# toverainc/willow-inference-server

Hardware: AMD Instinct MI355X
Metric: realtime_multiple (audio_ms / infer_ms), Whisper large-v2 beam=5, 3.84 s clip (higher is better)
Workload: dtype f16; 1 GPU; whisper-large beam=5 clip=3sec (3840 ms) batch=1/GPU, PCM resident in HBM -> ids on host; parallelism=1 independent replicas (utterance sharding, no data-path collective)

## Files before the change

### include/wis_hip.h

```cpp
#ifndef WIS_HIP_H
#define WIS_HIP_H

#include <stddef.h>
#include <stdint.h>

#ifdef __cplusplus
extern "C" {
#endif

#define WIS_ABI_VERSION 1

#define WIS_OK             0
#define WIS_E_ARG         -1
#define WIS_E_FORMAT      -2
#define WIS_E_NOMEM       -3
#define WIS_E_CHECKSUM    -4
#define WIS_E_HIP         -5
#define WIS_E_STATE       -6
#define WIS_E_UNSUPPORTED -7

#define WIS_SAMPLE_RATE 16000
#define WIS_N_FFT       400
#define WIS_HOP         160
#define WIS_N_MELS      80
// ... 38 lines not shown
  const int32_t* suppress_ids;       int32_t n_suppress;
  const int32_t* suppress_ids_begin; int32_t n_suppress_begin;
  const int32_t* lang_ids;           int32_t n_lang;
  int32_t decoder_weight_bits;
} wis_config_t;

#define WIS_DT_F32 0
#define WIS_DT_F16 1
typedef struct {
  const char* name;
  int32_t     dtype;
  int32_t     rank;
  int64_t     shape[4];
  uint64_t    offset;
} wis_tensor_t;

int  wis_model_create(const wis_config_t* cfg, const void* arena, size_t arena_bytes,
                      int arena_on_device, const wis_tensor_t* tensors, int n_tensors,
                      int device, wis_model_t** out);
void wis_model_destroy(wis_model_t* m);
size_t wis_model_device_bytes(const wis_model_t* m);
int  wis_model_clone(wis_model_t* parent, wis_model_t** out);

#define WIS_IN_MEL_HOST 0
#define WIS_IN_MEL_DEV  1
#define WIS_IN_PCM_HOST 2
#define WIS_IN_PCM_DEV  3

typedef struct {
  int32_t input_kind;
  int32_t beam_size;
  int32_t max_new_tokens;
  float   length_penalty;
  float   patience;
  int32_t suppress_blank;
  int32_t suppress_default;
  int32_t fixed_new_tokens;
  int32_t queue_depth;
  int32_t timestamps;
  int32_t max_initial_timestamp_index;
  int32_t no_speech_prob;
  float   repetition_penalty;
  int32_t no_repeat_ngram_size;
} wis_gen_opts_t;

int wis_generate(wis_model_t* m, const float* input, int B, const int32_t* prompt, int P,
                 const wis_gen_opts_t* opts, int32_t* out_ids, int32_t* out_len, float* out_score);

int wis_generate_draft(wis_model_t* m, const float* input, const int32_t* prompt, int P, const wis_gen_opts_t* opts,
                       const int32_t* draft, int n_draft, int32_t* out_ids, int32_t* out_len, float* out_score, int32_t* accepted);

int wis_generate_draft_beam(wis_model_t* m, const float* input, const int32_t* prompt, int P, const wis_gen_opts_t* opts,
                            const int32_t* draft_tok, const int32_t* draft_org, int n_steps,
                            int32_t* out_ids, int32_t* out_len, float* out_score, int32_t* accepted_steps);
int wis_last_trajectory(wis_model_t* m, int b, int32_t* tok, int32_t* org, int cap_steps, int32_t* n_steps);

int wis_last_no_speech_prob(wis_model_t* m, int B, float* out);

int wis_detect_language(wis_model_t* m, const float* input, int input_kind, int B, float* lang_probs);

int wis_debug_encode(wis_model_t* m, const float* input, int input_kind, int B, float* enc_out);
int wis_debug_logits(wis_model_t* m, const float* input, int input_kind, int B,
                     const int32_t* dec_in, int T, float* logits);
int wis_debug_logits_rows(wis_model_t* m, const float* input, int input_kind, int B,
                          const int32_t* dec_in, int T, int R, float* logits);
int wis_model_set_alignment_heads(wis_model_t* m, const int32_t* layer_head_pairs, int n);
int wis_align(wis_model_t* m, const float* input, int input_kind, int B, const int32_t* start_seq, int P,
              const int32_t* text, const int32_t* text_len, const int32_t* num_frames, int median_filter_width,
              int32_t* path_text, int32_t* path_time, int32_t* path_len, float* token_probs);
int wis_debug_align_matrix(wis_model_t* m, const float* input, int input_kind, int B, const int32_t* start_seq, int P,
                           const int32_t* text, const int32_t* text_len, const int32_t* num_frames, int median_filter_width, float* out);
int wis_align_last_timing(wis_model_t* m, float* ms);
int wis_op_dtw(int device, const float* x, int N, int M, int32_t* text_idx, int32_t* time_idx, int32_t* len);
int wis_op_align_matrix(int device, const float* q, const void* kx_f16, int T_tokens, int n_heads_sel, int T, int frames, int width, float* out);
int wis_debug_tree_logits(wis_model_t* m, const float* input, int input_kind, const int32_t* prompt, int P, int beam,
                          const int32_t* tok, const int32_t* org, int n_steps, float* logits);

int wis_debug_search(wis_model_t* m, const float* logits, int n_steps, int B, const wis_gen_opts_t* opts,
                     int32_t* out_ids, int32_t* out_len, float* out_score, int32_t* out_finish_step, int32_t* out_parent);

int wis_debug_handoff(wis_model_t* m, int raise_flag, int* retries, int* spin_disabled);

typedef struct {
  float logmel_ms, encoder_ms, crosskv_ms, prefill_ms, decode_ms, total_ms;
  int32_t decode_steps;
  int32_t decode_steps_needed;
} wis_timing_t;
int wis_last_timing(const wis_model_t* m, wis_timing_t* t);

int wis_debug_phase_cycles(wis_model_t* m, int B, int beam, int pos, uint64_t* out);

int wis_debug_timeline(wis_model_t* m, int B, int beam, int pos, int use_graph, uint64_t* out, int n_out);
int wis_debug_sampling_cycles(wis_model_t* m, uint64_t* out);

int wis_bench_weight_stream(wis_model_t* m, int M, int passes, float* total_ms, int* launches_per_pass,
                            double* bytes_per_pass);

int wis_dev_alloc(int device, size_t bytes, void** out);
int wis_dev_free(int device, void* p);
int wis_dev_h2d(int device, void* dst, const void* src, size_t bytes);
int wis_dev_d2h(int device, void* dst, const void* src, size_t bytes);
int wis_dev_sync(int device);
int wis_dev_copy_peer(int dst_device, void* dst, int src_device, const void* src, size_t bytes);

int wis_op_gemm(int device, const void* A_f16, int lda, const void* W_f16, const float* bias,
                const float* residual, void* C, int M, int N, int K, int flags);
int wis_op_layernorm(int device, const float* x, const float* gamma, const float* beta,
                     void* y_f16, int M, int d);
int wis_op_enc_attention(int device, const void* qk_f16, const void* vt_f16, void* out_f16,
                         int B, int T, int Tpad, int H);
int wis_op_enc_attention_ex(int device, const void* qk_f16, const void* vt_f16, void* out_f16,
                            int B, int T, int Tpad, int H, int form);
int wis_op_gemv(int device, const void* x, const float* gamma, const float* beta,
                const void* W_f16, const float* bias, void* y, int M, int N, int K, int flags);
int wis_op_gemv_cols(int device, const void* x_f16, const void* W_f16, const float* bias, void* y, void* y16,
                     int M, int N, int K, int flags, int cols);

int wis_op_dec_self_attn(int device, const float* q, const void* kc_f16, const void* vc_f16, const int32_t* pos, void* out_f16,
                         int M, int H, int ctx, int rpu, int sstride, int rmul);
int wis_op_dec_cross_attn(int device, const float* q, const void* kx_f16, const void* vt_f16, void* out_f16,
                          int B, int R, int H, int T, int chunks);
int wis_op_dec_cross_attn_folded(int device, const float* q_raw, const float* xres, const float* qcs, const float* qb,
                                 const void* kx_f16, const void* vt_f16, void* out_f16, int B, int R, int H, int T, int chunks);

int wis_op_dec_cross_attn_stat(int device, const float* q, const float* q2, const float* stat, const float* qcs, const float* qb,
                               const void* kx_f16, const void* vt_f16, void* out_f16, int B, int R, int H, int T, int chunks,
                               int out_mb, int kv_shared, int no_spin);
int wis_op_dec_self_attn_ex(int device, const float* q, const void* kc_f16, const void* vc_f16, const int32_t* pos, void* out_f16,
                            int M, int H, int ctx, int rpu, int sstride, int rmul, int nb, int out_mb,
                            const int32_t* anc, int w0, int aw, const int32_t* base);
int wis_op_gemv_qkv(int device, const float* x, const float* gamma, const float* beta, const void* W_f16, const float* bias,
                    const int32_t* slot, const int32_t* pos, float* q, void* kc_f16, void* vc_f16, int M, int d, int ctx);
int wis_op_gemv_out_cq(int device, const void* a_f16, const float* x0, const void* Wo_f16, const float* bo, const void* Wq_f16, const float* bq,
                       const float* gamma, const float* beta, float* x1, float* stat, float* q, float* q2, float* qcs, float* qb,
                       int M, int d, int force_frag);

int wis_op_mel_to_image(int device, const float* mel, void* img_f16, int B, int n_mels);
int wis_op_enc_conv(int device, int which, const void* img_f16, const void* W, int w_is_f16, const float* bias, const float* pos, void* out,
                    int B, int T, int Cin, int N);
int wis_op_enc_qkv(int device, const void* xn_f16, const void* W_f16, const float* bias, void* qk_f16, void* vt_f16, int B, int T, int H);
int wis_op_enc_crosskv(int device, const void* mem_f16, const void* W_f16, const float* bias, void* kx_f16, void* vt_f16, int B, int T, int H, int L,
                       int64_t kx_lstride, int64_t vt_lstride);
int wis_op_gemm_splitk_ln(int device, const void* A_f16, const void* W_f16, const float* bias, float* X, const float* gamma, const float* beta,
                          void* Y_f16, int M, int N, int K, int splits);

int wis_op_kv_reorder(int device, void* kc_f16, void* vc_f16, int64_t layer_stride_elems, int L, const int32_t* parent, const int32_t* step_u,
                      const int32_t* done, int B, int beam, int P, int ctx, int d);
int wis_op_kv_gather(int device, void* kc_f16, void* vc_f16, int64_t layer_stride_elems, int L, const int32_t* vstate, const int32_t* done,
                     int beam, int w0, int ctx, int d);
int wis_op_no_speech(int device, const float* logits, int ld, int B, int rs, int r0, int V, int ns, float* out);
int wis_op_lang_probs(int device, const float* logits, int ld, const int32_t* lang_ids, int n_lang, float* probs, int B);
int wis_op_greedy_rows(int device, const float* logits, int n_vocab, int n_vocab_pad, int eot, const float* bias_all, const float* bias_begin,
                       const int32_t* step_u, int B, int beam, int lr_b, int lr_j, int lr_off, const int32_t* rowmap, int32_t* tok_out, float* lp_out);

typedef struct wis_sv wis_sv_t;
typedef struct {
  int32_t conv_dim;
  int32_t n_conv_layers;
  int32_t conv_kernel[8], conv_stride[8];
  int32_t hidden_size, n_heads, n_layers, intermediate_size;
  int32_t num_conv_pos_embeddings, num_conv_pos_embedding_groups;
  int32_t num_buckets, max_bucket_distance;
  int32_t n_tdnn;
  int32_t tdnn_dim[8], tdnn_kernel[8], tdnn_dilation[8];
  int32_t xvector_output_dim;
  int64_t max_samples;
} wis_sv_config_t;
int    wis_sv_create(const wis_sv_config_t* cfg, const void* arena, size_t arena_bytes, int arena_on_device,
                     const wis_tensor_t* tensors, int n_tensors, int device, wis_sv_t** out);
void   wis_sv_destroy(wis_sv_t* sv);
size_t wis_sv_device_bytes(const wis_sv_t* sv);
int    wis_sv_embed(wis_sv_t* sv, const float* pcm, int64_t n, float* emb);
int    wis_sv_rel_buckets(int num_buckets, int max_distance, int first, int n, int32_t* out);
int    wis_debug_sv_taps(wis_sv_t* sv, const float* pcm, int64_t n, int tap, int layer, float* out, int64_t cap_floats,
                         int32_t* rows, int32_t* cols);
int    wis_op_sv_conv0(int device, const float* pcm, int64_t n, const float* w0, const float* gamma, const float* beta, void* y_f16);
int    wis_op_sv_posconv(int device, const float* x, const void* W_f16, const float* bias, float* out, int T);
int    wis_op_sv_attention(int device, const void* qkv_f16, const float* xin, const float* gw, const float* gb, const float* gconst,
                           const float* tab, int L, void* out_f16, int T);
int    wis_op_sv_layernorm(int device, const void* x, int in_f16, const float* gamma, const float* beta, void* y16, float* y32,
                           float* ws, void* ws16, float wl, int wmode, int M, int d);
int    wis_op_sv_xvector_tail(int device, const float* z, int ldz, int T, int n, const float* W_fe, const float* b_fe,
                              float* stats, float* emb);

#ifdef __cplusplus
}
#endif
#endif
```

### willow-inference-server_amd/csrc/dec_kernels.hip

```cpp
#include <string.h>
#include "common.hpp"
#include "kernels.hpp"

namespace wis {

__global__ void pack_gemv_kernel(const f16* __restrict__ W, f16* __restrict__ Wp, int N, int Npad, int K, int n_scale, float scale, int rows) {
  const int ksteps = K / 32;
  const size_t total = (size_t)Npad * ksteps * 4;
  for (size_t idx = (size_t)blockIdx.x * blockDim.x + threadIdx.x; idx < total; idx += (size_t)gridDim.x * blockDim.x) {
    const int row = (int)(idx % rows);
    size_t t = idx / rows;
    const int kq = (int)(t & 3); t >>= 2;
    const int ks = (int)(t % ksteps), nt = (int)(t / ksteps);
    const int n = rows * nt + row, k = 32 * ks + 8 * kq;
    f16x8 v;
    if (n < N) {
      v = *reinterpret_cast<const f16x8*>(W + (size_t)n * K + k);
      if (n < n_scale) {
#pragma unroll
        for (int j = 0; j < 8; ++j) v[j] = (f16)((float)v[j] * scale);
      }
    } else {
#pragma unroll
      for (int j = 0; j < 8; ++j) v[j] = (f16)0.f;
// ... 1744 lines not shown
      if (tid == 0) tl_end(prof);
      return;
    }
    if (pub) {
#pragma unroll
      for (int blk = 0; blk < NB; ++blk)
#pragma unroll
        for (int r4 = 0; r4 < 4; ++r4) own[l15][dhb + 16 * blk + r4] = o_[blk][r4];
      if (wave == NKW && kq == 0) { own[l15][64] = Mc; own[l15][65] = Lc; }
    }
    __syncthreads();
    stamp(pf, 5);
    for (int item = tid; item < R * 32; item += NTHR) {
      const int r = item >> 5, dp = item & 31;
      float2 ml[CM], ov[CM];
      unsigned spins = 0;
      for (;;) {
        bool ok = true;
#pragma unroll
        for (int cc = 0; cc < CM - 1; ++cc) {
          if (cc < C - 1) {
            const gran_t* gp = gbase + ((size_t)cc * 8 + r) * 66;
            const gran_t g0 = ld_gran(gp + 64), g1 = ld_gran(gp + 65), g2 = ld_gran(gp + 2 * dp), g3 = ld_gran(gp + 2 * dp + 1);
            ok = ok & ((unsigned)(g0 >> 32) == tag) & ((unsigned)(g1 >> 32) == tag) & ((unsigned)(g2 >> 32) == tag) & ((unsigned)(g3 >> 32) == tag);
            ml[cc] = make_float2(__uint_as_float((unsigned)g0), __uint_as_float((unsigned)g1));
            ov[cc] = make_float2(__uint_as_float((unsigned)g2), __uint_as_float((unsigned)g3));
          }
        }
        if (ok) break;
        if (++spins > CA_SPIN_LIMIT) { atomicOr(epoch, 1u); break; }
        __builtin_amdgcn_s_sleep(1);
      }
      float M_ = own[r][64];
#pragma unroll
      for (int cc = 0; cc < CM - 1; ++cc) if (cc < C - 1) M_ = fmaxf(M_, ml[cc].x);
      float L = 0.f, O0 = 0.f, O1 = 0.f;
#pragma unroll
      for (int cc = 0; cc < CM - 1; ++cc) {
        if (cc < C - 1) {
          const float w = __expf(ml[cc].x - M_);
          L = fmaf(ml[cc].y, w, L); O0 = fmaf(ov[cc].x, w, O0); O1 = fmaf(ov[cc].y, w, O1);
        }
      }
      {
        const float w = __expf(own[r][64] - M_);
        L = fmaf(own[r][65], w, L); O0 = fmaf(own[r][2 * dp], w, O0); O1 = fmaf(own[r][2 * dp + 1], w, O1);
      }
      const float inv = 1.0f / L;
      typedef _Float16 f16x2 __attribute__((ext_vector_type(2)));
      const f16x2 o2 = {(f16)(O0 * inv), (f16)(O1 * inv)};
      *reinterpret_cast<f16x2*>(out + (out_mb ? xf_index(b * R + r, h * 64 + 2 * dp, out_mb) : (size_t)(b * R + r) * d + h * 64 + 2 * dp)) = o2;
    }
    if (tid == 0) __hip_atomic_store(epoch + 1 + b * H + h, tag, __ATOMIC_RELAXED, __HIP_MEMORY_SCOPE_AGENT);
    stamp(pf, 6);
    if (tid == 0) tl_end(prof);
    return;
  }
  float* pbase = part + ((size_t)(b * H + h) * C) * R * 66;
  if (pub) {
    float* pp = pbase + ((size_t)c * R + l15) * 66;
#pragma unroll
    for (int blk = 0; blk < NB; ++blk)
#pragma unroll
      for (int r4 = 0; r4 < 4; ++r4) st_sc1(pp + dhb + 16 * blk + r4, o_[blk][r4]);
    if (wave == NKW && kq == 0) { st_sc1(pp + 64, Mc); st_sc1(pp + 65, Lc); }
  }
  asm volatile("s_waitcnt vmcnt(0)" ::: "memory");
  __syncthreads();
  stamp(pf, 5);
  if (tid == 0) {
    const unsigned prev = __hip_atomic_fetch_add(counters + b * H + h, 1u, __ATOMIC_RELAXED, __HIP_MEMORY_SCOPE_AGENT);
    const int last = (prev == (unsigned)(C - 1));
    if (last) {
      __hip_atomic_store(counters + b * H + h, 0u, __ATOMIC_RELAXED, __HIP_MEMORY_SCOPE_AGENT);
      __builtin_amdgcn_fence(__ATOMIC_ACQUIRE, "agent");
    }
    s_last = last;
  }
  __syncthreads();
  if (tid == 0) tl_end(prof);
  if (!s_last) return;
  for (int item = tid; item < R * 32; item += NTHR) {
    const int r = item >> 5, dp = item & 31;
    float2 ml[CM], ov[CM];
#pragma unroll
    for (int cc = 0; cc < CM; ++cc) {
      if (cc < C) {
        const float* pp = pbase + ((size_t)cc * R + r) * 66;
        ml[cc] = *reinterpret_cast<const float2*>(pp + 64);
        ov[cc] = *reinterpret_cast<const float2*>(pp + 2 * dp);
      }
    }
    float M_ = -INFINITY;
#pragma unroll
    for (int cc = 0; cc < CM; ++cc) if (cc < C) M_ = fmaxf(M_, ml[cc].x);
    float L = 0.f, O0 = 0.f, O1 = 0.f;
#pragma unroll
    for (int cc = 0; cc < CM; ++cc) {
      if (cc < C) {
        const float w = __expf(ml[cc].x - M_);
        L = fmaf(ml[cc].y, w, L); O0 = fmaf(ov[cc].x, w, O0); O1 = fmaf(ov[cc].y, w, O1);
      }
    }
    const float inv = 1.0f / L;
    typedef _Float16 f16x2 __attribute__((ext_vector_type(2)));
    const f16x2 o2 = {(f16)(O0 * inv), (f16)(O1 * inv)};
    *reinterpret_cast<f16x2*>(out + (out_mb ? xf_index(b * R + r, h * 64 + 2 * dp, out_mb) : (size_t)(b * R + r) * d + h * 64 + 2 * dp)) = o2;
  }
  stamp(pf, 6);
}

int launch_dec_cross_attn(hipStream_t st, const CrossAttnP& p) {
  const int B = p.B, R = p.R, H = p.H, d = p.d, T = p.T, Tpad = p.Tpad, chunks = p.chunks, xres_is_stat = p.xres_is_stat;
  const float* const xres = p.xres;
  if (xres && (!p.qcs || !p.qb || R > 8 || d > (xres_is_stat ? 2048 : 1280))) { set_error("dec_cross_attn: folded query needs column sums, bias, R <= 8 and d <= 1280 (2048 from partials)"); return WIS_E_ARG; }
  if (xres_is_stat && !xres) { set_error("dec_cross_attn: the fold from partials needs the row partials"); return WIS_E_ARG; }
  if (R < 1 || R > 16 || chunks < 1 || chunks > 16) { set_error("dec_cross_attn: R=%d chunks=%d unsupported", R, chunks); return WIS_E_UNSUPPORTED; }
  if (H > 63 || d > 65535 || T > 65535) { set_error("dec_cross_attn: H=%d d=%d T=%d beyond the packed shape arguments", H, d, T); return WIS_E_UNSUPPORTED; }
  const int CL = cdiv(cdiv(T, chunks), 32) * 32;
  if ((CL != 128 && CL != 256) || CL * chunks > Tpad) { set_error("dec_cross_attn: %d chunks of %d keys unsupported (Tpad %d)", chunks, CL, Tpad); return WIS_E_UNSUPPORTED; }
  const int used = cdiv(T, CL);
  static const int env_spin = getenv("WIS_CA_SPIN") ? atoi(getenv("WIS_CA_SPIN")) : 1;
  const bool spin = env_spin && p.gran && p.epoch && B * H <= CA_SPIN_MAX_BH && CL == 256 && used >= 2 && used <= 6 && R <= 8;
#define WIS_CA(TPWv, CMv, FOLDv, SPINv) hipLaunchKernelGGL((dec_cross_attn_kernel<TPWv, CMv, FOLDv, SPINv>), dim3(used, H, B), dim3(256), 0, st, p.q, p.kx, p.vt, xres, p.q2, p.epoch, \
                                                  (R | (H << 8) | (CL << 14) | (used << 24)), (d | (T << 16)), (Tpad | (p.kv_shared ? (1 << 30) : 0)), p.out, p.part, p.counters, p.prof, p.out_mb, p.qcs, p.qb, p.gran)
  if (xres_is_stat) {
    const bool small = (long)B * H * used <= 256;
    static const int ca_rs = getenv("WIS_CA_RS") ? atoi(getenv("WIS_CA_RS")) : 2;
    if (ca_rs && (!small || ca_rs >= 2) && CL == 256 && used <= 6 && R <= 8 && d <= 1280) {
#define WIS_CA_RS(SPINv, NTv) hipLaunchKernelGGL((dec_cross_attn_rs_kernel<SPINv, NTv, 2>), dim3(used, H, B), dim3(256), 0, st, p.q, p.kx, p.vt, xres, p.q2, p.epoch, \
                                                        (R | (H << 8) | (CL << 14) | (used << 24)), (d | (T << 16)), (Tpad | (p.kv_shared ? (1 << 30) : 0)), p.out, p.part, p.counters, p.prof, p.out_mb, p.qcs, p.qb, p.gran)
      if (spin) { if (small) WIS_CA_RS(true, true); else WIS_CA_RS(true, false); }
      else { if (small) WIS_CA_RS(false, true); else WIS_CA_RS(false, false); }
#undef WIS_CA_RS
      return WIS_OK;
    }
    static const bool fold4 = !(getenv("WIS_CA_FOLD4") && atoi(getenv("WIS_CA_FOLD4")) == 0);
    const bool f4 = fold4 && !small && R <= 8;
    if (spin) { if (small) WIS_CA(4, 6, 3, true); else if (f4) WIS_CA(4, 6, 4, true); else WIS_CA(4, 6, 2, true); }
    else if (CL <= 128) WIS_CA(2, 16, 2, false);
    else if (used <= 6) { if (small) WIS_CA(4, 6, 3, false); else if (f4) WIS_CA(4, 6, 4, false); else WIS_CA(4, 6, 2, false); } else WIS_CA(4, 16, 2, false);
  }
  else if (spin) { if (xres) WIS_CA(4, 6, 1, true); else WIS_CA(4, 6, 0, true); }
  else if (xres) { if (CL <= 128) WIS_CA(2, 16, 1, false); else if (used <= 6) WIS_CA(4, 6, 1, false); else WIS_CA(4, 16, 1, false); }
  else { if (CL <= 128) WIS_CA(2, 16, 0, false); else if (used <= 6) WIS_CA(4, 6, 0, false); else WIS_CA(4, 16, 0, false); }
#undef WIS_CA
  return WIS_OK;
}

__device__ __forceinline__ bool better(float av, int ai, float bv, int bi) { return av > bv || (av == bv && ai < bi); }
__device__ __forceinline__ bool better_b(float av, int ai, float bv, int bi) { return (av > bv) | ((av == bv) & (ai < bi)); }
__device__ __forceinline__ void take_better(float& v, int& i, float ov, int oi) { const bool t = better_b(ov, oi, v, i); v = t ? ov : v; i = t ? oi : i; }

template <bool TS>
__global__ __launch_bounds__(256) void logit_stats_kernel(const float* __restrict__ logits, const float* __restrict__ bias_all,
                                                          const float* __restrict__ bias_begin, const int* __restrict__ step_u,
                                                          float* __restrict__ st_max, float* __restrict__ st_sum,
                                                          float* __restrict__ st_val, int* __restrict__ st_idx, SampleCfg cfg,
                                                          int lr_b, int lr_j, int lr_off, unsigned long long* prof, const int* __restrict__ rowmap,
                                                          const int* __restrict__ ts_desc) {
  constexpr int PT = 16;
  const int tid = threadIdx.x, lane = tid & 63, wave = tid >> 6;
  const int sc = blockIdx.x * 4 + wave, m = blockIdx.y, b = m / cfg.beam;
  unsigned long long* pf = (blockIdx.x == 0 && blockIdx.y == 0 && tid == 0) ? prof : nullptr;
  stamp(pf, 0);
  const int step = step_u[b];
  const int SL = cdiv(cfg.n_vocab, STAT_SUB);
  const int lo = sc * SL, hi = (lo + SL < cfg.n_vocab) ? lo + SL : cfg.n_vocab;
  const int jb = m - b * cfg.beam;
  const float* row = logits + (size_t)(b * lr_b + (rowmap ? rowmap[jb] : jb) * lr_j + lr_off) * cfg.n_vocab_pad;
  const bool first = (step == 0) && cfg.suppress_blank;
  const bool mask_eot = cfg.fixed_new > 0 && step < cfg.fixed_new;
  const bool force_eot = cfg.fixed_new > 0 && step >= cfg.fixed_new;

  float vals[PT]; u64 keys[PT];
  float lv[PT], la[PT], lb[PT];
  int r0l = 0, r0h = 0, r1l = 0, r1h = 0, r2l = 0, r2h = 0;
  if constexpr (TS) {
    const int* dsc = ts_desc + m * TS_DESC_INTS;
    r0l = dsc[0]; r0h = dsc[1]; r1l = dsc[2]; r1h = dsc[3]; r2l = dsc[4]; r2h = dsc[5];
  }
#pragma unroll
  for (int i = 0; i < PT; ++i) {
    const int nidx = lo + lane + 64 * i;
    const int cidx = nidx < hi ? nidx : hi - 1;
    lv[i] = row[cidx]; lb[i] = bias_begin[cidx]; la[i] = bias_all ? bias_all[cidx] : 0.f;
  }
  float mx = -INFINITY;
#pragma unroll
  for (int i = 0; i < PT; ++i) {
    const int nidx = lo + lane + 64 * i;
    float v = lv[i] + la[i];
    v = first ? v + lb[i] : v;
    bool dead = (nidx >= hi) | (mask_eot & (nidx == cfg.eot)) | (force_eot & (nidx != cfg.eot));
    if constexpr (TS) dead = dead | ((nidx >= r0l) & (nidx < r0h)) | ((nidx >= r1l) & (nidx < r1h)) | ((nidx >= r2l) & (nidx < r2h));
    v = dead ? -INFINITY : v;
    vals[i] = v; keys[i] = nidx < hi ? sel_key(v, nidx) : 0ull; mx = fmaxf(mx, v);
  }
  stamp(pf, 1);
  mx = wave_max(mx);
  float sum = 0.f;
  if (mx > -INFINITY) {
#pragma unroll
    for (int i = 0; i < PT; ++i) sum += __expf(vals[i] - mx);
  }
  sum = wave_sum(sum);
  if (lane == 0) { st_max[m * STAT_SUB + sc] = mx; st_sum[m * STAT_SUB + sc] = sum; }
  stamp(pf, 2);
  u64 prev = ~0ull;
  for (int rnd = 0; rnd < cfg.n_cand; ++rnd) {
    u64 t[PT];
#pragma unroll
    for (int i = 0; i < PT; ++i) t[i] = keys[i] < prev ? keys[i] : 0ull;
#pragma unroll
    for (int w = PT / 2; w >= 1; w >>= 1)
#pragma unroll
      for (int i = 0; i < w; ++i) t[i] = key_max(t[i], t[i + w]);
    const u64 best = wave_max_key(t[0]);
    if (lane == 0) {
      st_val[((size_t)m * STAT_SUB + sc) * cfg.n_cand + rnd] = best ? key_value(best) : -INFINITY;
      st_idx[((size_t)m * STAT_SUB + sc) * cfg.n_cand + rnd] = best ? key_index(best) : 0x7fffffff;
    }
    prev = best;
  }
  stamp(pf, 3);
}
int launch_logit_stats(hipStream_t st, const float* logits, const float* bias_all, const float* bias_begin, const int* step_u,
                       float* st_max, float* st_sum, float* st_val, int* st_idx, int B, const SampleCfg& cfg, int lr_b, int lr_j, int lr_off,
                       unsigned long long* prof, const int* rowmap, const int* ts_desc) {
  if (cdiv(cfg.n_vocab, STAT_SUB) > 16 * 64) { set_error("logit_stats: vocab too large"); return WIS_E_UNSUPPORTED; }
  if (ts_desc) hipLaunchKernelGGL(logit_stats_kernel<true>, dim3(STAT_SUB / 4, B * cfg.beam), dim3(256), 0, st, logits, bias_all, bias_begin, step_u,
                                  st_max, st_sum, st_val, st_idx, cfg, lr_b, lr_j, lr_off, prof, rowmap, ts_desc);
  else hipLaunchKernelGGL(logit_stats_kernel<false>, dim3(STAT_SUB / 4, B * cfg.beam), dim3(256), 0, st, logits, bias_all, bias_begin, step_u,
                          st_max, st_sum, st_val, st_idx, cfg, lr_b, lr_j, lr_off, prof, rowmap, nullptr);
  return WIS_OK;
}

__device__ __forceinline__ float block_max_256(float v, float* red) {
  v = wave_max(v);
  const int lane = threadIdx.x & 63, wave = threadIdx.x >> 6;
  __syncthreads();
  if (lane == 0) red[wave] = v;
  __syncthreads();
  return fmaxf(fmaxf(red[0], red[1]), fmaxf(red[2], red[3]));
}
__device__ __forceinline__ float block_sum_256(float v, float* red) {
  v = wave_sum(v);
  const int lane = threadIdx.x & 63, wave = threadIdx.x >> 6;
  __syncthreads();
  if (lane == 0) red[wave] = v;
  __syncthreads();
  return (red[0] + red[1]) + (red[2] + red[3]);
}
__global__ __launch_bounds__(256) void ts_rules_kernel(const float* __restrict__ logits, const float* __restrict__ bias_all,
                                                       const float* __restrict__ bias_begin, const int* __restrict__ step_u,
                                                       const int* __restrict__ alive, SampleCfg cfg, int no_ts, int max_init,
                                                       int lr_b, int lr_j, int lr_off, int* __restrict__ ts_desc) {
  __shared__ float red[4];
  const int tid = threadIdx.x, m = blockIdx.x, b = m / cfg.beam, jb = m - b * cfg.beam;
  const int V = cfg.n_vocab, tb = no_ts + 1;
  int step = step_u[b];
  step = step < cfg.max_new ? step : cfg.max_new;
  const bool force_eot = cfg.fixed_new > 0 && step >= cfg.fixed_new;
  int* dsc = ts_desc + m * TS_DESC_INTS;
  if (force_eot) {
    if (tid < TS_DESC_INTS) dsc[tid] = (tid == 7) ? step : 0;
    return;
  }
  const bool first = (step == 0) && cfg.suppress_blank;
  const bool mask_eot = cfg.fixed_new > 0 && step < cfg.fixed_new;
  int r0l = no_ts, r0h = no_ts + 1, r1l = 0, r1h = 0, r2l = 0, r2h = 0;
  if (step == 0) {
    r0l = 0; r0h = tb;
    if (max_init >= 0 && tb + max_init + 1 < V) { r1l = tb + max_init + 1; r1h = V; }
  } else {
    const int* hist = alive + (size_t)m * cfg.max_new;
    const int tk = tid < step ? hist[tid] : -1;
    const float lastpos = block_max_256(tk >= tb ? (float)tid : -1.f, red);
    const int last = hist[step - 1];
    const bool last_ts = last >= tb;
    const bool pen_ts = step < 2 || hist[step - 2] >= tb;
    if (last_ts) { if (pen_ts) { r1l = tb; r1h = V; } else { r1l = 0; r1h = cfg.eot; } }
    if (lastpos >= 0.f) {
      const int t_ts = hist[(int)lastpos];
      const int t_last = (last_ts && !pen_ts) ? t_ts : t_ts + 1;
      r2l = tb; r2h = t_last;
    }
  }
  const float* row = logits + (size_t)(b * lr_b + jb * lr_j + lr_off) * cfg.n_vocab_pad;
  auto value = [&](int i) -> float {
    float v = row[i] + (bias_all ? bias_all[i] : 0.f);
    v = first ? v + bias_begin[i] : v;
    const bool dead = (mask_eot & (i == cfg.eot)) | ((i >= r0l) & (i < r0h)) | ((i >= r1l) & (i < r1h)) | ((i >= r2l) & (i < r2h));
    return dead ? -INFINITY : v;
  };
  float tmx = -INFINITY;
  for (int i = tid; i < tb; i += 256) tmx = fmaxf(tmx, value(i));
  float smx = -INFINITY;
  for (int i = tb + tid; i < V; i += 256) smx = fmaxf(smx, value(i));
  tmx = block_max_256(tmx, red);
  smx = block_max_256(smx, red);
  float ssum = 0.f;
  if (smx > -INFINITY)
    for (int i = tb + tid; i < V; i += 256) ssum += expf(value(i) - smx);
  ssum = block_sum_256(ssum, red);
  const float lse = smx > -INFINITY ? smx + logf(ssum) : -INFINITY;
  const bool ts_wins = lse > tmx;
  if (ts_wins) { r0l = 0; r0h = tb; }
  if (tid == 0) {
    dsc[0] = r0l; dsc[1] = r0h; dsc[2] = r1l; dsc[3] = r1h; dsc[4] = r2l; dsc[5] = r2h; dsc[6] = ts_wins ? 1 : 0; dsc[7] = step;
  }
}
int launch_ts_rules(hipStream_t st, const float* logits, const float* bias_all, const float* bias_begin, const BeamState& bs, int B,
                    const SampleCfg& cfg, int no_ts, int max_init, int lr_b, int lr_j, int lr_off, int* ts_desc) {
  if (cfg.max_new > 256 || no_ts + 1 >= cfg.n_vocab) { set_error("ts_rules: config out of range"); return WIS_E_UNSUPPORTED; }
  hipLaunchKernelGGL(ts_rules_kernel, dim3(B * cfg.beam), dim3(256), 0, st, logits, bias_all, bias_begin, bs.step_u, bs.alive, cfg, no_ts, max_init,
                     lr_b, lr_j, lr_off, ts_desc);
  return WIS_OK;
}

__global__ __launch_bounds__(256) void rep_rules_kernel(float* __restrict__ logits, const int* __restrict__ step_u, const int* __restrict__ done,
                                                        const int* __restrict__ alive, SampleCfg cfg, float penalty, int ngram,
                                                        int lr_b, int lr_j, int lr_off) {
  __shared__ int4 sh4[64];
  int* sh = reinterpret_cast<int*>(sh4);
  const int tid = threadIdx.x, m = blockIdx.x, b = m / cfg.beam, jb = m - b * cfg.beam;
  if (done[b]) return;
  int L = step_u[b];
  L = L < cfg.max_new ? L : cfg.max_new;
  if (L <= 0 || (cfg.fixed_new > 0 && L >= cfg.fixed_new)) return;
  const int V = cfg.n_vocab;
  int tk = tid < L ? alive[(size_t)m * cfg.max_new + tid] : -1;
  tk = (tk >= 0 && tk < V) ? tk : -1;
  sh[tid] = tk;
  __syncthreads();
  float* row = logits + (size_t)(b * lr_b + jb * lr_j + lr_off) * cfg.n_vocab_pad;
  if (penalty != 1.f) {
    bool dup = false;
    for (int i = 0; i < L; i += 4) {
      const int4 h = sh4[i >> 2];
      dup = dup | ((h.x == tk) & (i < tid)) | ((h.y == tk) & (i + 1 < tid)) | ((h.z == tk) & (i + 2 < tid)) | ((h.w == tk) & (i + 3 < tid));
    }
    if (tk >= 0 && !dup) { const float x = row[tk]; row[tk] = x < 0.f ? x * penalty : __fdiv_rn(x, penalty); }
  }
  if (ngram >= 1 && L >= ngram) {
    __syncthreads();
    bool hit = tid <= L - ngram;
    const int i0 = hit ? tid : 0, tail = L - ngram + 1;
    for (int q = 0; q < ngram - 1; ++q) hit = hit & (sh[i0 + q] == sh[tail + q]);
    const int t = sh[i0 + ngram - 1];
    if (hit && t >= 0) row[t] = -INFINITY;
  }
}
int launch_rep_rules(hipStream_t st, float* logits, const BeamState& bs, int B, const SampleCfg& cfg, float penalty, int ngram, int lr_b, int lr_j, int lr_off) {
  if (cfg.max_new > 256 || !(penalty > 0.f) || ngram < 0) { set_error("rep_rules: config out of range"); return WIS_E_UNSUPPORTED; }
  hipLaunchKernelGGL(rep_rules_kernel, dim3(B * cfg.beam), dim3(256), 0, st, logits, bs.step_u, bs.done, bs.alive, cfg, penalty, ngram, lr_b, lr_j, lr_off);
  return WIS_OK;
}

__global__ __launch_bounds__(256) void no_speech_kernel(const float* __restrict__ logits, int ld, int rs, int r0, int V, int ns, float* __restrict__ out) {
  __shared__ float red[4];
  const int b = blockIdx.x, tid = threadIdx.x;
  const float* row = logits + (size_t)(b * rs + r0) * ld;
  float mx = -INFINITY;
  for (int i = tid; i < V; i += 256) mx = fmaxf(mx, row[i]);
  mx = block_max_256(mx, red);
  float s = 0.f;
  for (int i = tid; i < V; i += 256) s += expf(row[i] - mx);
  s = block_sum_256(s, red);
  if (tid == 0) out[b] = expf(row[ns] - mx) / s;
}
int launch_no_speech(hipStream_t st, const float* logits, int ld, int B, int rs, int r0, int V, int ns, float* out) {
  if (ns < 0 || ns >= V) { set_error("no_speech: token %d outside the vocabulary", ns); return WIS_E_ARG; }
  hipLaunchKernelGGL(no_speech_kernel, dim3(B), dim3(256), 0, st, logits, ld, rs, r0, V, ns, out);
  return WIS_OK;
}

__global__ __launch_bounds__(64) void greedy_pick_kernel(const float* __restrict__ st_max, const float* __restrict__ st_sum, const float* __restrict__ st_val,
                                                         const int* __restrict__ st_idx, int n_cand, int V, int* __restrict__ tok_out, float* __restrict__ lp_out) {
  const int m = blockIdx.x, lane = threadIdx.x;
  const float smx = st_max[m * STAT_SUB + lane], ssm = st_sum[m * STAT_SUB + lane];
  const float v = st_val[((size_t)m * STAT_SUB + lane) * n_cand];
  const int ix = st_idx[((size_t)m * STAT_SUB + lane) * n_cand];
  const float M_ = wave_max(smx);
  const float S = wave_sum(smx > -INFINITY ? ssm * __expf(smx - M_) : 0.f);
  const float lse = M_ + logf(S);
  const int tk = ix > V - 1 ? V - 1 : ix;
  const u64 best = wave_max_key(sel_key(v > -INFINITY ? v - lse : -INFINITY, tk));
  if (lane == 0) { tok_out[m] = key_index(best); lp_out[m] = key_value(best); }
}
int launch_greedy_pick(hipStream_t st, const float* st_max, const float* st_sum, const float* st_val, const int* st_idx, int rows, const SampleCfg& cfg, int* tok_out, float* lp_out) {
  hipLaunchKernelGGL(greedy_pick_kernel, dim3(rows), dim3(64), 0, st, st_max, st_sum, st_val, st_idx, cfg.n_cand, cfg.n_vocab, tok_out, lp_out);
  return WIS_OK;
}

__device__ __forceinline__ void publish_step(const BeamState& bs) {
  __threadfence();
  const unsigned B = gridDim.x;
  const unsigned n = atomicAdd(bs.tick, 1u) + 1u;
  if (n % B != 0u) return;
  __threadfence();
  const unsigned steps = n / B;
  const unsigned done = (unsigned)__hip_atomic_load(bs.all_done, __ATOMIC_RELAXED, __HIP_MEMORY_SCOPE_AGENT);
  const unsigned gen = __hip_atomic_load(bs.tick + 1, __ATOMIC_RELAXED, __HIP_MEMORY_SCOPE_AGENT);
  const unsigned gu = bs.giveup ? (__hip_atomic_load(bs.giveup, __ATOMIC_RELAXED, __HIP_MEMORY_SCOPE_AGENT) != 0u ? 1u : 0u) : 0u;
  const unsigned long long now = (unsigned long long)__builtin_amdgcn_s_memrealtime();
  if (steps == 1u) __hip_atomic_store(bs.host + HP_STAMP0, now, __ATOMIC_RELAXED, __HIP_MEMORY_SCOPE_SYSTEM);
  __hip_atomic_store(bs.host + HP_STAMP, now, __ATOMIC_RELAXED, __HIP_MEMORY_SCOPE_SYSTEM);
  if (done >= B && atomicCAS(bs.tick + 2, 0u, steps) == 0u) {
    __hip_atomic_store(bs.host + HP_DONE_STEP, (unsigned long long)steps, __ATOMIC_RELAXED, __HIP_MEMORY_SCOPE_SYSTEM);
    __hip_atomic_store(bs.host + HP_DONE_STAMP, now, __ATOMIC_RELAXED, __HIP_MEMORY_SCOPE_SYSTEM);
  }
  const unsigned long long rec = ((unsigned long long)(gen & 0xFFFFu) << 48) | ((unsigned long long)(steps & 0xFFFFu) << 32) | ((unsigned long long)gu << 16) | (done & 0xFFFFu);
  __hip_atomic_store(bs.host + HP_REC, rec, __ATOMIC_RELEASE, __HIP_MEMORY_SCOPE_SYSTEM);
}

template <int PSL>
__global__ __launch_bounds__(256) void beam_step_kernel(const float* __restrict__ st_max, const float* __restrict__ st_sum,
                                                        const float* __restrict__ st_val, const int* __restrict__ st_idx,
                                                        BeamState bs, RowMeta rm, int P, int ctx, SampleCfg cfg, unsigned long long* prof) {
  constexpr int HPT = (MAX_R * 256 + 255) / 256;
  __shared__ float lse[MAX_R], s_cum[MAX_R];
  __shared__ float cand_v[MAX_CAND]; __shared__ int cand_word[MAX_CAND]; __shared__ int cand_org[MAX_CAND];
  __shared__ int nb_src[MAX_R]; __shared__ int nb_tok[MAX_R]; __shared__ float nb_cum[MAX_R];
  __shared__ int hyp_src[MAX_R]; __shared__ int hyp_slot[MAX_R]; __shared__ int hyp_n[MAX_R]; __shared__ int n_newhyp;
  __shared__ int s_finished;
  __shared__ int sh_alive[MAX_R * 256];
  const int b = blockIdx.x, tid = threadIdx.x, lane = tid & 63, wave = tid >> 6;
  unsigned long long* pf = (b == 0 && tid == 0) ? prof : nullptr;
  stamp(pf, 0);
  const int k = cfg.beam, NC = cfg.n_cand, V = cfg.n_vocab;
  const int r0 = b * k, per_row = STAT_SUB * NC, total = k * per_row;
  float pv_[PSL]; int pi_[PSL];
#pragma unroll
  for (int u = 0; u < PSL; ++u) {
    const int e = tid + 256 * u, ce = e < total ? e : total - 1;
    const float v = st_val[(size_t)r0 * per_row + ce]; const int ix = st_idx[(size_t)r0 * per_row + ce];
    pv_[u] = e < total ? v : -INFINITY; pi_[u] = e < total ? ix : 0x7fffffff;
  }
  float smx[2], ssm[2];
#pragma unroll
  for (int j2 = 0; j2 < 2; ++j2) {
    const int j = wave + 4 * j2, mrow = r0 + (j < k ? j : 0);
    smx[j2] = st_max[mrow * STAT_SUB + lane]; ssm[j2] = st_sum[mrow * STAT_SUB + lane];
  }
  const float my_cum = tid < k ? bs.cum[r0 + tid] : 0.f;
  int hist_tok[HPT];
#pragma unroll
  for (int u = 0; u < HPT; ++u) {
    const int i = tid + 256 * u, j = i >> 8, t = i & 255;
    const int cj = j < k ? j : k - 1, ct = t < cfg.max_new ? t : cfg.max_new - 1;
    hist_tok[u] = bs.alive[(size_t)(r0 + cj) * cfg.max_new + ct];
  }
  const int done_b = bs.done[b];
  const int step = bs.step_u[b];
  const int nh0 = bs.n_hyp[b];
  if (done_b) { if (tid == 0) publish_step(bs); return; }

  stamp(pf, 1);
#pragma unroll
  for (int u = 0; u < HPT; ++u) { const int i = tid + 256 * u; if (i < MAX_R * 256) sh_alive[i] = hist_tok[u]; }
  if (tid < k) s_cum[tid] = my_cum;
#pragma unroll
  for (int j2 = 0; j2 < 2; ++j2) {
    const int j = wave + 4 * j2;
    const float M_ = wave_max(smx[j2]);
    const float S = wave_sum(smx[j2] > -INFINITY ? ssm[j2] * __expf(smx[j2] - M_) : 0.f);
    if (lane == 0 && j < k) lse[j] = M_ + logf(S);
  }
  __syncthreads();
  stamp(pf, 2);
  u64 pk[PSL];
  u64 lbest = 0ull;
  const float inv_per_row = 1.0f / (float)per_row;
#pragma unroll
  for (int u = 0; u < PSL; ++u) {
    const int e = tid + 256 * u;
    int j = (int)(((float)e + 0.5f) * inv_per_row);
    j = j < k ? j : k - 1;
    const float v = pv_[u];
    const float sc_ = (v - lse[j]) + s_cum[j];
    int tk = pi_[u]; tk = tk > V - 1 ? V - 1 : tk;
    pk[u] = e < total ? sel_key(v > -INFINITY ? sc_ : -INFINITY, (j << 20) | tk) : 0ull;
    lbest = key_max(lbest, pk[u]);
  }
  stamp(pf, 3);
  __shared__ u64 wcand[4 * MAX_CAND];
  for (int rnd = 0; rnd < NC; ++rnd) {
    const u64 wb = wave_max_key(lbest);
    if (lane == 0) wcand[wave * NC + rnd] = wb;
#pragma unroll
    for (int u = 0; u < PSL; ++u) pk[u] = pk[u] == wb ? 0ull : pk[u];
    u64 t[PSL];
#pragma unroll
    for (int u = 0; u < PSL; ++u) t[u] = pk[u];
#pragma unroll
    for (int w = PSL / 2; w >= 1; w >>= 1)
#pragma unroll
      for (int u = 0; u < w; ++u) t[u] = key_max(t[u], t[u + w]);
    lbest = t[0];
  }
  if (tid < MAX_CAND) { cand_v[tid] = -INFINITY; cand_word[tid] = V - 1; cand_org[tid] = 0; }
  __syncthreads();
  if (tid < 4 * NC) {
    const u64 mine = wcand[tid];
    int rank = 0;
#pragma unroll
    for (int m2 = 0; m2 < 4 * MAX_CAND; ++m2) rank += (m2 < 4 * NC && wcand[m2] > mine) ? 1 : 0;
    if (mine != 0ull && rank < NC) {
      const int bi = key_index(mine);
      cand_v[rank] = key_value(mine); cand_word[rank] = bi & 0xFFFFF; cand_org[rank] = (bi >> 20) & 0x7FF;
    }
  }
  __syncthreads();

  stamp(pf, 4);
  if (tid == 0) {
    const bool is_last = (step + 1 >= cfg.max_new);
    int nh = nh0, second = k, newh = 0; bool top_finished = false;
    for (int kk = 0; kk < k; ++kk) {
      int next = kk;
      const bool eos = cand_word[kk] == cfg.eot;
      if (eos || is_last) {
        if (kk == 0) top_finished = true;
        if (nh < cfg.max_hyp) {
          hyp_src[newh] = kk; hyp_slot[newh] = nh; hyp_n[newh] = eos ? step : step + 1;
          bs.hyp_score[b * cfg.max_hyp + nh] = cand_v[kk];
          bs.hyp_len[b * cfg.max_hyp + nh] = hyp_n[newh];
          ++newh; ++nh;
        }
        for (int j = second; j < NC; ++j)
          if (cand_word[j] != cfg.eot) { next = j; second = j + 1; break; }
      }
      nb_src[kk] = next; nb_tok[kk] = cand_word[next]; nb_cum[kk] = cand_v[next];
    }
    n_newhyp = newh;
    bs.n_hyp[b] = nh;
    bool fin = is_last;
    if (!fin) fin = cfg.allow_early_exit ? (top_finished && nh >= cfg.early_exit_hyps) : (nh >= cfg.max_candidates);
    s_finished = fin ? 1 : 0;
  }
  __syncthreads();

  stamp(pf, 5);
  const int hist = step;
  const int npos = P - 1 + step + 1;
  for (int hh = 0; hh < n_newhyp; ++hh) {
    const int kk = hyp_src[hh], org = cand_org[kk], n = hyp_n[hh];
    int* dst = bs.hyp_tok + ((size_t)b * cfg.max_hyp + hyp_slot[hh]) * cfg.max_new;
    for (int t = tid; t < n; t += 256) dst[t] = (t < hist) ? sh_alive[org * 256 + t] : cand_word[kk];
  }
  if (s_finished) {
    __syncthreads();
    __threadfence_block();
    if (tid == 0) {
      const int nh = bs.n_hyp[b];
      int best = 0; float bsc = -INFINITY;
      for (int i = 0; i < nh; ++i) {
        float s = bs.hyp_score[b * cfg.max_hyp + i];
        const int n = bs.hyp_len[b * cfg.max_hyp + i];
        if (cfg.length_penalty != 0.f) s /= powf((float)n, cfg.length_penalty);
        if (s > bsc) { bsc = s; best = i; }
      }
      cand_org[0] = best;
      bs.out_len[b] = bs.hyp_len[b * cfg.max_hyp + best];
      bs.out_score[b] = bsc;
      bs.done[b] = 1;
      hp_out_len(bs.host)[b] = bs.hyp_len[b * cfg.max_hyp + best];
      hp_out_score(bs.host)[b] = bsc;
    }
    __syncthreads();
    const int best = cand_org[0], n = bs.hyp_len[b * cfg.max_hyp + best];
    const int* src = bs.hyp_tok + ((size_t)b * cfg.max_hyp + best) * cfg.max_new;
    int* hids = hp_out_ids(bs.host) + (size_t)b * cfg.max_new;
    for (int t = tid; t < n; t += 256) { const int v = src[t]; bs.out_ids[(size_t)b * cfg.max_new + t] = v; hids[t] = v; }
    __threadfence_system();
    __syncthreads();
    if (tid == 0) { atomicAdd(bs.all_done, 1); publish_step(bs); }
    return;
  }
  stamp(pf, 7);
  for (int j = 0; j < k; ++j) {
    const int org = cand_org[nb_src[j]];
    int* al = bs.alive + (size_t)(r0 + j) * cfg.max_new;
    for (int t = tid; t < hist; t += 256) al[t] = sh_alive[org * 256 + t];
    if (tid == 0) {
      al[hist] = nb_tok[j];
      bs.parent[r0 + j] = (step == 0) ? r0 : r0 + org;
      { int* tr = bs.traj + ((size_t)(b * 256 + step) * MAX_R + j) * 2; tr[0] = nb_tok[j]; tr[1] = org; }
      bs.cum[r0 + j] = nb_cum[j];
      rm.tok[r0 + j] = nb_tok[j];
      rm.pos[r0 + j] = npos;
      rm.slot[r0 + j] = r0 + j;
    }
  }
  if (tid == 0) bs.step_u[b] = step + 1;
  __syncthreads();
  if (tid == 0) publish_step(bs);
  stamp(pf, 8);
}
int launch_beam_step(hipStream_t st, const float* st_max, const float* st_sum, const float* st_val, const int* st_idx,
                     const BeamState& bs, const RowMeta& rm, int B, int P, int ctx, const SampleCfg& cfg, unsigned long long* prof) {
  if (cfg.beam > MAX_R || cfg.n_cand > MAX_CAND || cfg.max_new > 256 || ctx > 512 || cfg.n_vocab > (1 << 20)) { set_error("beam_step: config out of range"); return WIS_E_UNSUPPORTED; }
  if (cfg.beam * STAT_SUB * cfg.n_cand <= 16 * 256) hipLaunchKernelGGL(beam_step_kernel<16>, dim3(B), dim3(256), 0, st, st_max, st_sum, st_val, st_idx, bs, rm, P, ctx, cfg, prof);
  else hipLaunchKernelGGL(beam_step_kernel<32>, dim3(B), dim3(256), 0, st, st_max, st_sum, st_val, st_idx, bs, rm, P, ctx, cfg, prof);
  return WIS_OK;
}

constexpr int VS_PERM = 8, VS_BASE = 16, VS_PATH = 32, VS_PATH_W = 32, VS_INTS = VS_PATH + MAX_R * VS_PATH_W;
__global__ __launch_bounds__(64) void draft_match_kernel(BeamState bs, const int* __restrict__ draft, int n_draft, int k, int* __restrict__ vs, int book) {
  __shared__ int org_r[MAX_R], tok_r[MAX_R], perm_prev[MAX_R], old_base[MAX_R], old_path[MAX_R][VS_PATH_W];
  const int tid = threadIdx.x;
  if (bs.done[0]) return;
  const int s = bs.step_u[0] - 1;
  const int t = vs[2];
  if (tid < k) {
    const int* tr = bs.traj + ((size_t)s * MAX_R + tid) * 2;
    tok_r[tid] = tr[0]; org_r[tid] = tr[1]; perm_prev[tid] = vs[VS_PERM + tid]; old_base[tid] = vs[VS_BASE + tid];
  }
  for (int e = tid; e < k * VS_PATH_W; e += 64) old_path[e / VS_PATH_W][e % VS_PATH_W] = vs[VS_PATH + e];
  __syncthreads();
  if (book) {
    for (int e = tid; e < k * VS_PATH_W; e += 64) {
      const int j = e / VS_PATH_W, u = e % VS_PATH_W, pj = org_r[j];
      if (u < t) vs[VS_PATH + e] = old_path[pj][u];
      else if (u == t) vs[VS_PATH + e] = perm_prev[pj];
    }
    if (tid < k) vs[VS_BASE + tid] = old_base[org_r[tid]];
  }
  if (tid == 0) {
    bool ok = s >= 0 && s < n_draft;
    int pn[MAX_R]; unsigned used = 0;
    if (ok) {
      const int* dr = draft + (size_t)s * MAX_R * 2;
      for (int j = 0; j < k && ok; ++j) {
        const int want_org = perm_prev[org_r[j]];
        int hit = -1;
        for (int i = 0; i < k; ++i) if (!((used >> i) & 1u) && dr[2 * i] == tok_r[j] && dr[2 * i + 1] == want_org) { hit = i; break; }
        if (hit < 0) ok = false; else { pn[j] = hit; used |= 1u << hit; }
      }
    }
    if (ok) { for (int j = 0; j < k; ++j) vs[VS_PERM + j] = pn[j]; vs[0] = s + 1; }
    else bs.done[0] = 2;
    if (book) vs[2] = t + 1;
  }
}
int launch_draft_match(hipStream_t st, const BeamState& bs, const int* draft, int n_draft, int beam, int* vstate, int book) {
  hipLaunchKernelGGL(draft_match_kernel, dim3(1), dim3(64), 0, st, bs, draft, n_draft, beam, vstate, book);
  return WIS_OK;
}
__global__ __launch_bounds__(256) void kv_gather_kernel(f16* __restrict__ kc, f16* __restrict__ vc, size_t lstride, const int* __restrict__ vs, const int* __restrict__ done,
                                                        int k, int w0, int ctx, int d) {
  const int lk = blockIdx.y, tid = threadIdx.x;
  const int nwin = vs[2];
  if (done[0] == 1 || nwin <= 0) return;
  f16* cache = ((lk & 1) ? vc : kc) + (size_t)(lk >> 1) * lstride;
  const int c8 = d >> 3, npos = w0 + nwin;
  for (int p = blockIdx.x; p < npos; p += gridDim.x) {
    int par[MAX_R];
#pragma unroll
    for (int j = 0; j < MAX_R; ++j) par[j] = j < k ? (p < w0 ? vs[VS_BASE + j] : vs[VS_PATH + j * VS_PATH_W + (p - w0)]) : j;
    for (int ch = tid; ch < c8; ch += 256) {
      u32x4 v[MAX_R];
#pragma unroll
      for (int j = 0; j < MAX_R; ++j) if (j < k && par[j] != j) v[j] = *reinterpret_cast<const u32x4*>(cache + ((size_t)par[j] * ctx + p) * d + ch * 8);
      asm volatile("s_waitcnt vmcnt(0)" ::: "memory");
#pragma unroll
      for (int j = 0; j < MAX_R; ++j) if (j < k && par[j] != j) *reinterpret_cast<u32x4*>(cache + ((size_t)j * ctx + p) * d + ch * 8) = v[j];
    }
  }
}
int launch_kv_gather(hipStream_t st, f16* kc, f16* vc, size_t layer_stride, int L, const int* vstate, const int* done, int beam, int w0, int ctx, int d) {
  hipLaunchKernelGGL(kv_gather_kernel, dim3(8, 2 * L), dim3(256), 0, st, kc, vc, layer_stride, vstate, done, beam, w0, ctx, d);
  return WIS_OK;
}

__global__ __launch_bounds__(256) void kv_reorder_kernel(f16* __restrict__ kc, f16* __restrict__ vc, size_t lstride, const int* __restrict__ parent,
                                                         const int* __restrict__ step_u, const int* __restrict__ done, int k, int P, int ctx, int d) {
  const int b = blockIdx.z, lk = blockIdx.y, tid = threadIdx.x;
  if (k < 2) return;
  const int r0 = b * k;
  const int dn = done[b], st = step_u[b];
  int par[MAX_R];
#pragma unroll
  for (int j = 0; j < MAX_R; ++j) par[j] = parent[r0 + (j < k ? j : 0)];
  bool ident = true;
#pragma unroll
  for (int j = 0; j < MAX_R; ++j) { if (j < k) ident = ident & (par[j] == r0 + j); else par[j] = r0 + j; }
  if (dn | (int)ident) return;
  const int npos = P - 1 + st;
  f16* cache = ((lk & 1) ? vc : kc) + (size_t)(lk >> 1) * lstride;
  const int c8 = d >> 3;
  for (int p = blockIdx.x; p < npos; p += gridDim.x) {
    for (int ch = tid; ch < c8; ch += 256) {
      u32x4 v[MAX_R];
#pragma unroll
      for (int j = 0; j < MAX_R; ++j) if (j < k && par[j] != r0 + j) v[j] = *reinterpret_cast<const u32x4*>(cache + ((size_t)par[j] * ctx + p) * d + ch * 8);
      asm volatile("s_waitcnt vmcnt(0)" ::: "memory");
#pragma unroll
      for (int j = 0; j < MAX_R; ++j) if (j < k && par[j] != r0 + j) *reinterpret_cast<u32x4*>(cache + ((size_t)(r0 + j) * ctx + p) * d + ch * 8) = v[j];
    }
  }
}
int launch_kv_reorder(hipStream_t st, f16* kc, f16* vc, size_t layer_stride, int L, const BeamState& bs, int B, int beam, int P, int ctx, int d) {
  if (beam < 2) return WIS_OK;
  if (beam > MAX_R) { set_error("kv_reorder: beam %d > %d", beam, MAX_R); return WIS_E_UNSUPPORTED; }
  hipLaunchKernelGGL(kv_reorder_kernel, dim3(8, 2 * L, B), dim3(256), 0, st, kc, vc, layer_stride, bs.parent, bs.step_u, bs.done, beam, P, ctx, d);
  return WIS_OK;
}

__global__ void lang_probs_kernel(const float* __restrict__ logits, int ld, const int* __restrict__ lang_ids, int n_lang, float* __restrict__ probs) {
  const int b = blockIdx.x, lane = threadIdx.x;
  const float* row = logits + (size_t)b * ld;
  float mx = -INFINITY;
  for (int i = lane; i < n_lang; i += 64) mx = fmaxf(mx, row[lang_ids[i]]);
  mx = wave_max(mx);
  float s = 0.f;
  for (int i = lane; i < n_lang; i += 64) s += __expf(row[lang_ids[i]] - mx);
  s = wave_sum(s);
  for (int i = lane; i < n_lang; i += 64) probs[(size_t)b * n_lang + i] = __expf(row[lang_ids[i]] - mx) / s;
}
int launch_lang_probs(hipStream_t st, const float* logits, int ld, const int* lang_ids, int n_lang, float* probs, int B) {
  hipLaunchKernelGGL(lang_probs_kernel, dim3(B), dim3(64), 0, st, logits, ld, lang_ids, n_lang, probs);
  return WIS_OK;
}

}
```

### willow-inference-server_amd/csrc/generate.hip

```cpp

struct SampleCtx {
  wis_model* m; hipStream_t st;
  int B, P, beam;
  SampleCfg sc; const float* bias_all;
  bool ts; int ts_max_init;
  float rep_pen = 1.f; int rep_ngram = 0;
  bool rep() const { return rep_pen != 1.f || rep_ngram != 0; }
};
static int resolve_rep_opts(const wis_gen_opts_t* o, SampleCtx* g) {
  const float p = o->repetition_penalty; const int n = o->no_repeat_ngram_size;
  if (!std::isfinite(p) || p < 0.f) { set_error("repetition_penalty %g: a finite value > 0 (1 or 0: off)", (double)p); return WIS_E_ARG; }
  if (n < 0) { set_error("no_repeat_ngram_size %d: >= 0 (0: off)", n); return WIS_E_ARG; }
  g->rep_pen = p == 0.f ? 1.f : p; g->rep_ngram = n;
  return WIS_OK;
}
struct GenCtx : SampleCtx {
  const float* input; const int32_t* prompt; const wis_gen_opts_t* o;
  const int32_t *draft, *draft_org; int n_draft;
  int max_new; float patience;
  std::chrono::steady_clock::time_point t0;
  int sot_row;
  bool drafting, beam_draft;
};

static int make_gen_ctx(wis_model* m, const float* input, int B, const int32_t* prompt, int P, const wis_gen_opts_t* o,
                        const int32_t* draft, int n_draft, const int32_t* draft_org, GenCtx* out) {
  const wis_config_t& c = m->cfg;
  GenCtx& g = *out;
  g.m = m; g.st = m->st; g.input = input; g.prompt = prompt; g.o = o; g.draft = draft; g.draft_org = draft_org; g.n_draft = n_draft; g.B = B; g.P = P;
  const int beam = g.beam = o->beam_size < 1 ? 1 : o->beam_size;
  WIS_RET(check_batch(m, B, beam));
  WIS_RET(check_patience(beam, o->patience));
  if (P < 1 || P > 16 || B * P > MAX_ROWS) { set_error("prompt length %d unsupported (1..16, B*P <= %d)", P, MAX_ROWS); return WIS_E_UNSUPPORTED; }
  int max_new = o->max_new_tokens > 0 ? o->max_new_tokens : std::min(c.n_text_ctx / 2, c.n_text_ctx - P);
  if (max_new > MAX_STEPS) max_new = MAX_STEPS;
  if (P - 1 + max_new > c.n_text_ctx) max_new = c.n_text_ctx - (P - 1);
  g.max_new = max_new;
  for (int i = 0; i < B * P; ++i) if (prompt[i] < 0 || prompt[i] >= c.n_vocab) { set_error("prompt token %d out of range", prompt[i]); return WIS_E_ARG; }
  WIS_RET(resolve_rep_opts(o, &g));
  g.t0 = std::chrono::steady_clock::now();
  g.sc = make_sample_cfg(m, o, beam, max_new, &g.patience);
  g.bias_all = o->suppress_default ? m->bias_all : nullptr;
  const bool drafting = g.drafting = draft != nullptr && n_draft > 0;
  const bool beam_draft = g.beam_draft = drafting && draft_org != nullptr;
  if (drafting && B != 1) { set_error("wis_generate_draft: one utterance per call (got B = %d)", B); return WIS_E_UNSUPPORTED; }
  if (drafting && !beam_draft && beam != 1) { set_error("wis_generate_draft: beam_size 1 (a beam search is drafted by its trajectory: wis_generate_draft_beam)"); return WIS_E_UNSUPPORTED; }
  g.ts = o->timestamps != 0;
  g.ts_max_init = o->max_initial_timestamp_index < 0 ? -1 : o->max_initial_timestamp_index;
  if (g.ts && draft != nullptr) { set_error("timestamps: not available for drafted decodes (wis_generate_draft / wis_generate_draft_beam)"); return WIS_E_UNSUPPORTED; }
  if (g.rep() && draft != nullptr) { set_error("repetition_penalty / no_repeat_ngram_size: not available for drafted decodes (wis_generate_draft / wis_generate_draft_beam)"); return WIS_E_UNSUPPORTED; }
  int sot_row = -1;
  if (o->no_speech_prob && !drafting) {
    for (int i = 0; i < P; ++i) if (prompt[i] == c.sot) { sot_row = i; break; }
    for (int b = 1; b < B && sot_row >= 0; ++b) if (prompt[b * P + sot_row] != c.sot) sot_row = -1;
    if (sot_row < 0) { set_error("no_speech_prob: the prompts hold no common <|startoftranscript|> position"); return WIS_E_ARG; }
  }
  g.sot_row = sot_row;
  if (beam_draft && (beam < 2 || n_draft > MAX_STEPS)) { set_error("wis_generate_draft_beam: beam_size >= 2 and at most 256 draft steps (got %d, %d)", beam, n_draft); return WIS_E_ARG; }
  if (drafting) for (int i = 0; i < n_draft * (beam_draft ? beam : 1); ++i) if (draft[i] < 0 || draft[i] >= c.n_vocab) { set_error("draft token %d out of range", draft[i]); return WIS_E_ARG; }
  if (beam_draft) for (int i = 0; i < n_draft * beam; ++i) if (draft_org[i] < 0 || draft_org[i] >= beam) { set_error("draft origin %d outside [0, beam_size)", draft_org[i]); return WIS_E_ARG; }
  return WIS_OK;
}

static int stage_search(const GenCtx& g) {
  wis_model* m = g.m; const int B = g.B, P = g.P, beam = g.beam;
  WIS_RET(init_beam_state(m, B, beam));
  m->last_B = B; m->last_beam = beam;
  if (!g.drafting || g.beam_draft) {
    std::vector<int> tok(B * P), pos(B * P), slot(B * P), ls(B * P);
    for (int b = 0; b < B; ++b) for (int i = 0; i < P; ++i) { tok[b * P + i] = g.prompt[b * P + i]; pos[b * P + i] = i; slot[b * P + i] = b * beam; ls[b * P + i] = b * beam; }
    WIS_RET(upload_rows(m, tok, pos, slot, ls, false));
  }
  if (m->overrun_left) { WIS_HIP_CHECK(hipMemsetAsync(m->ca_epoch, 0, 4, g.st)); m->overrun_left = false; }
  __atomic_store_n(&m->h_prog[HP_REC], 0ull, __ATOMIC_RELAXED);
  m->h_prog[HP_DONE_STEP] = 0; m->h_prog[HP_DONE_STAMP] = 0; m->h_prog[HP_STAMP0] = 0;
  return WIS_OK;
}

static int front_half(const GenCtx& g) {
  wis_model* m = g.m; hipStream_t st = g.st; const int B = g.B;
  static const bool one_stream = getenv("WIS_ONE_STREAM") != nullptr;
  static const bool two_streams = getenv("WIS_TWO_STREAMS") != nullptr;
  const bool alone = g_active_calls[m->device & 63].load(std::memory_order_relaxed) <= 1;
  hipStream_t se = (one_stream || !(alone || two_streams)) ? st : m->st_enc;
  if (se != st) WIS_HIP_CHECK(hipStreamWaitEvent(se, m->ev_ckv, 0));
  WIS_HIP_CHECK(hipEventRecord(m->ev[0], se));
  WIS_RET(stage_input(m, g.input, g.o->input_kind, B, se));
  WIS_HIP_CHECK(hipEventRecord(m->ev[1], se));
  WIS_RET(run_encoder(m, B, se));
  WIS_HIP_CHECK(hipEventRecord(m->ev[2], se));
  if (se != st) { WIS_HIP_CHECK(hipEventRecord(m->ev_enc, se)); WIS_HIP_CHECK(hipStreamWaitEvent(st, m->ev_enc, 0)); }
  WIS_RET(run_cross_kv(m, B));
  WIS_HIP_CHECK(hipEventRecord(m->ev[3], st));
  WIS_HIP_CHECK(hipEventRecord(m->ev_ckv, st));
  return WIS_OK;
}

struct LogitRows { int b, j, off; };
enum { TAIL_TAPS = 1, TAIL_NO_CACHE = 2 };
static int sampling_tail(const SampleCtx& g, LogitRows rows, int flags) {
  wis_model* m = g.m; hipStream_t st = g.st; const wis_config_t& c = m->cfg;
  const int lr_b = rows.b, lr_j = rows.j, lr_off = rows.off;
  unsigned long long* prof = (WIS_TAPS && (flags & TAIL_TAPS)) ? m->d_prof + (size_t)c.n_dec_layers * 8 * 16 : nullptr;
  if (g.rep()) WIS_RET(launch_rep_rules(st, m->logits, m->bs, g.B, g.sc, g.rep_pen, g.rep_ngram, lr_b, lr_j, lr_off));
  if (g.ts) WIS_RET(launch_ts_rules(st, m->logits, g.bias_all, m->bias_begin, m->bs, g.B, g.sc, c.no_timestamps, g.ts_max_init, lr_b, lr_j, lr_off, m->ts_desc));
  WIS_RET(launch_logit_stats(st, m->logits, g.bias_all, m->bias_begin, m->bs.step_u, m->st_max, m->st_sum, m->st_val, m->st_idx, g.B, g.sc, lr_b, lr_j, lr_off, prof ? prof + 16 : nullptr,
                             nullptr, g.ts ? m->ts_desc : nullptr));
  WIS_RET(launch_beam_step(st, m->st_max, m->st_sum, m->st_val, m->st_idx, m->bs, m->rm, g.B, g.P, c.n_text_ctx, g.sc, prof));
  if (!(flags & TAIL_NO_CACHE)) WIS_RET(launch_kv_reorder(st, m->kc_all, m->vc_all, m->kv_layer_stride, c.n_dec_layers, m->bs, g.B, g.beam, g.P, c.n_text_ctx, c.d_model));
  return WIS_OK;
}

struct Seed {
  int steps = 1;
  bool spec_done = false;
  bool beam_fin = false;
  std::vector<int> spec_gen; float spec_cum = 0.f; int spec_len = 0;
  int accepted = 0;
};

struct TicketScope {
  wis_model* m; bool spin_call;
  explicit TicketScope(wis_model* mm) : m(mm), spin_call(mm->spin_now) { m->spin_now = false; }
  ~TicketScope() { m->spin_now = spin_call; }
};

static int reseed_tick(wis_model* m, int steps) {
  unsigned* tk = m->h_pin->reseed_tick;
  tk[0] = (unsigned)steps; tk[1] = m->gen; tk[2] = 0; tk[3] = 0;
  WIS_HIP_CHECK(hipMemcpyAsync(m->bs.tick, tk, 16, hipMemcpyHostToDevice, m->st));
  return WIS_OK;
}

static void pack_traj(int* hd, const int32_t* tok, const int32_t* org, int n, int k) {
  for (int s_ = 0; s_ < n; ++s_) for (int j = 0; j < k; ++j) { hd[(s_ * MAX_R + j) * 2] = tok[s_ * k + j]; hd[(s_ * MAX_R + j) * 2 + 1] = org[s_ * k + j]; }
}

static int seed_prefill(const GenCtx& g) {
  wis_model* m = g.m; const wis_config_t& c = m->cfg; const int B = g.B, P = g.P;
  WIS_RET(dec_forward(m, B * P, P, B, true, g.beam, 0));
  if (g.sot_row >= 0) WIS_RET(launch_no_speech(g.st, m->logits, m->n_vocab_pad, B, P, g.sot_row, c.n_vocab, c.no_speech, m->d_nsp));
  return sampling_tail(g, {P, 0, P - 1}, TAIL_TAPS);
}

static int fill_tree_window(const int* hd, int s0, int Rw, int k, int P, std::vector<int>& tok, std::vector<int>& pos, std::vector<int>& slot, std::vector<int>& ls, int* ha) {
  const int Mreal = k * Rw, Mpad = cdiv(Mreal, 16) * 16;
  tok.assign(Mpad, 0); pos.assign(Mpad, 0); slot.assign(Mpad, 0); ls.assign(Mpad, 0);
  for (int t = 0; t < Rw; ++t) for (int j = 0; j < k; ++j) {
    const int s_ = s0 + t, r = t * k + j;
    tok[r] = hd[((s_ - 1) * MAX_R + j) * 2]; pos[r] = P - 1 + s_; slot[r] = j; ls[r] = j;
    int a = j;
    for (int sp = s_; sp >= s0; --sp) { ha[r * ANC_W + (sp - s0)] = a; a = hd[((sp - 1) * MAX_R + a) * 2 + 1]; }
    for (int u = t + 1; u < ANC_W; ++u) ha[r * ANC_W + u] = ha[r * ANC_W + t];
  }
  for (int r = Mreal; r < Mpad; ++r) {
    tok[r] = tok[Mreal - 1]; pos[r] = pos[Mreal - 1]; slot[r] = slot[Mreal - 1]; ls[r] = ls[Mreal - 1];
    for (int u = 0; u < ANC_W; ++u) ha[r * ANC_W + u] = ha[(Mreal - 1) * ANC_W + u];
  }
  return Mpad;
}

static int seed_beam_draft(const GenCtx& g, Seed* sd) {
  wis_model* m = g.m; hipStream_t st = g.st; const wis_config_t& c = m->cfg; PinnedScratch* hp = m->h_pin;
  const int P = g.P, beam = g.beam, max_new = g.max_new, ctx = c.n_text_ctx;
  const SampleCfg& sc = g.sc;
  const int k = beam;
  const int nd = std::min(g.n_draft, max_new - 1);
  int* hd = hp->draft;
  pack_traj(hd, g.draft, g.draft_org, nd, k);
  int* hv = hp->vstate;
  for (int i = 0; i < 32; ++i) hv[i] = 0;
  for (int j = 0; j < MAX_R; ++j) { hv[DRAFT_VS_PERM + j] = j; hv[DRAFT_VS_BASE + j] = j; }
  if (nd > 0) WIS_HIP_CHECK(hipMemcpyAsync(m->d_draft, hd, (size_t)nd * MAX_R * 2 * 4, hipMemcpyHostToDevice, st));
  WIS_HIP_CHECK(hipMemcpyAsync(m->d_vstate, hv, 32 * 4, hipMemcpyHostToDevice, st));
  WIS_RET(dec_forward(m, P, P, 1, true, beam, 0));
  WIS_RET(sampling_tail(g, {P, 0, P - 1}, 0));
  WIS_RET(launch_draft_match(st, m->bs, m->d_draft, nd, k, m->d_vstate, 0));
  const int RW = std::min(ANC_W, MAX_ROWS / k);
  const int s_last = std::min(nd, max_new - 1);
  int* ha = hp->anc;
  int* hb = hp->base;
  int* hw2 = hp->path_reset;
  int done_flag = 0, step_dev = 0;
  int pinv[MAX_R];
  for (int j = 0; j < MAX_R; ++j) pinv[j] = j;
  for (int s0 = 1;; ) {
    const int Rw = std::min(RW, s_last - s0 + 1);
    if (Rw >= 1) {
      std::vector<int> tok, pos, slot, ls;
      const int Mpad = fill_tree_window(hd, s0, Rw, k, P, tok, pos, slot, ls, ha);
      for (int r = 0; r < Mpad; ++r) hb[r] = pinv[ha[r * ANC_W]];
      const RowMeta rm_search = m->rm;
      m->rm = m->rm_win;
      int rc = upload_rows(m, tok, pos, slot, ls, false, &hp->win_rows);
      if (!rc && (hipMemcpyAsync(m->d_anc, ha, (size_t)Mpad * ANC_W * 4, hipMemcpyHostToDevice, st) != hipSuccess ||
                  hipMemcpyAsync(m->d_base, hb, (size_t)Mpad * 4, hipMemcpyHostToDevice, st) != hipSuccess)) { set_error("draft window: ancestor table upload failed"); rc = WIS_E_HIP; }
      TreeWin tw{m->d_anc, P - 1 + s0, ANC_W}; tw.base = m->d_base;
      if (!rc) rc = dec_forward(m, Mpad, 16, Mpad / 16, true, 1, 0, &tw);
      m->rm = rm_search;
      WIS_RET(rc);
      hw2[0] = 0; for (int j = 0; j < MAX_R; ++j) hw2[1 + j] = j;
      WIS_HIP_CHECK(hipMemcpyAsync(m->d_vstate + 2, hw2, 4, hipMemcpyHostToDevice, st));
      WIS_HIP_CHECK(hipMemcpyAsync(m->d_vstate + DRAFT_VS_BASE, hw2 + 1, MAX_R * 4, hipMemcpyHostToDevice, st));
      for (int t = 0; t < Rw; ++t) {
        WIS_RET(launch_logit_stats(st, m->logits, g.bias_all, m->bias_begin, m->bs.step_u, m->st_max, m->st_sum, m->st_val, m->st_idx, 1, sc, beam, 1, t * k, nullptr, m->d_vstate + DRAFT_VS_PERM));
        WIS_RET(launch_beam_step(st, m->st_max, m->st_sum, m->st_val, m->st_idx, m->bs, m->rm, 1, P, ctx, sc));
        WIS_RET(launch_draft_match(st, m->bs, m->d_draft, nd, k, m->d_vstate, 1));
      }
      WIS_RET(launch_kv_gather(st, m->kc_all, m->vc_all, m->kv_layer_stride, c.n_dec_layers, m->d_vstate, m->bs.done, beam, P - 1 + s0, ctx, c.d_model));
    }
    WIS_HIP_CHECK(hipMemcpyAsync(hv, m->d_vstate, 16 * 4, hipMemcpyDeviceToHost, st));
    WIS_HIP_CHECK(hipMemcpyAsync(&hp->win_done, m->bs.done, 4, hipMemcpyDeviceToHost, st));
    WIS_HIP_CHECK(hipMemcpyAsync(&hp->win_step, m->bs.step_u, 4, hipMemcpyDeviceToHost, st));
    WIS_HIP_CHECK(hipStreamSynchronize(st));
    done_flag = hp->win_done; step_dev = hp->win_step;
    if (Rw < 1 || done_flag != 0) break;
    for (int j = 0; j < k; ++j) { const int n_ = hv[DRAFT_VS_PERM + j]; if (n_ >= 0 && n_ < k) pinv[n_] = j; }
    s0 += Rw;
  }
  sd->accepted = hv[0];
  __atomic_store_n(&m->h_prog[HP_REC], 0ull, __ATOMIC_RELAXED);
  if (done_flag == 1) {
    sd->beam_fin = true; sd->steps = step_dev + 1;
  } else {
    sd->steps = step_dev;
    if (sd->steps < 1) { set_error("wis_generate_draft_beam: verification completed no step"); return WIS_E_STATE; }
    WIS_RET(reseed_tick(m, sd->steps));
    WIS_HIP_CHECK(hipMemsetAsync(m->bs.done, 0, 4, st));
  }
  return WIS_OK;
}

static int seed_greedy_draft(const GenCtx& g, Seed* sd) {
  wis_model* m = g.m; hipStream_t st = g.st; const wis_config_t& c = m->cfg; PinnedScratch* hp = m->h_pin;
  const int P = g.P, max_new = g.max_new;
  const int32_t* draft = g.draft;
  const int nd = std::min(g.n_draft, max_new - 1);
  std::vector<int> seq(P + nd);
  for (int i = 0; i < P; ++i) seq[i] = g.prompt[i];
  for (int i = 0; i < nd; ++i) seq[P + i] = draft[i];
  static const int env_rows = getenv("WIS_DRAFT_ROWS") ? atoi(getenv("WIS_DRAFT_ROWS")) : 0;
  const int R = (env_rows >= 16 && env_rows <= MAX_ROWS) ? env_rows / 16 * 16 : MAX_ROWS;
  bool stop = false; int n_acc = 0;
  for (int t0 = 0; t0 < P + nd && !stop; t0 += R) {
    const int rows = std::min(R, P + nd - t0);
    const int f = std::max(P - 1 - t0, 0), nv = rows - f;
    const int Mp = rows > 16 ? cdiv(rows, 16) * 16 : rows;
    std::vector<int> tok(Mp), pos(Mp), slot(Mp, 0), ls(Mp, 0);
    for (int i = 0; i < Mp; ++i) { const int ii = std::min(i, rows - 1); tok[i] = seq[t0 + ii]; pos[i] = t0 + ii; }
    WIS_RET(upload_rows(m, tok, pos, slot, ls));
    if (rows > 16) {
      WIS_HIP_CHECK(hipMemsetAsync(m->d_anc, 0, (size_t)Mp * 16 * 4, st));
      const TreeWin tw{m->d_anc, t0, 16};
      WIS_RET(dec_forward(m, Mp, 16, Mp / 16, nv > 0, 1, 0, &tw));
    } else
    WIS_RET(dec_forward(m, rows, rows, 1, nv > 0, 1, 0));
    if (nv <= 0) continue;
    int* hv = hp->vstep;
    for (int i = 0; i < nv; ++i) hv[i] = t0 + f + i - (P - 1);
    WIS_HIP_CHECK(hipMemcpyAsync(m->vstep, hv, (size_t)nv * 4, hipMemcpyHostToDevice, st));
    WIS_RET(launch_logit_stats(st, m->logits, g.bias_all, m->bias_begin, m->vstep, m->st_max, m->st_sum, m->st_val, m->st_idx, nv, g.sc, 1, 0, f));
    WIS_RET(launch_greedy_pick(st, m->st_max, m->st_sum, m->st_val, m->st_idx, nv, g.sc, m->pick_tok, m->pick_lp));
    int* ht = hp->pick_tok; float* hl = hp->pick_lp;
    WIS_HIP_CHECK(hipMemcpyAsync(ht, m->pick_tok, (size_t)nv * 4, hipMemcpyDeviceToHost, st));
    WIS_HIP_CHECK(hipMemcpyAsync(hl, m->pick_lp, (size_t)nv * 4, hipMemcpyDeviceToHost, st));
    WIS_HIP_CHECK(hipStreamSynchronize(st));
    for (int i = 0; i < nv && !stop; ++i) {
      const int gi = hv[i];
      sd->spec_cum = hl[i] + sd->spec_cum;
      sd->spec_gen.push_back(ht[i]);
      const bool eos = ht[i] == c.eot, is_last = gi + 1 >= max_new;
      if (eos || is_last) { sd->spec_done = true; sd->spec_len = eos ? gi : gi + 1; stop = true; }
      else if (gi < nd && ht[i] == draft[gi]) ++n_acc;
      else stop = true;
    }
  }
  sd->accepted = n_acc;
  const int steps = sd->steps = (int)sd->spec_gen.size();
  if (steps < 1) { set_error("wis_generate_draft: verification produced no token"); return WIS_E_STATE; }
  if (!sd->spec_done) {
    int* hs = hp->hist;
    for (int t = 0; t < steps; ++t) hs[t] = sd->spec_gen[t];
    WIS_HIP_CHECK(hipMemcpyAsync(m->bs.alive, hs, (size_t)steps * 4, hipMemcpyHostToDevice, st));
    auto& hw = hp->seed;
    hw.step = steps; hw.tok = sd->spec_gen.back(); hw.pos = P - 1 + steps; hw.slot = 0; hw.cum = sd->spec_cum;
    WIS_HIP_CHECK(hipMemcpyAsync(m->bs.step_u, &hw.step, 4, hipMemcpyHostToDevice, st));
    WIS_HIP_CHECK(hipMemcpyAsync(m->rm.tok, &hw.tok, 4, hipMemcpyHostToDevice, st));
    WIS_HIP_CHECK(hipMemcpyAsync(m->rm.pos, &hw.pos, 4, hipMemcpyHostToDevice, st));
    WIS_HIP_CHECK(hipMemcpyAsync(m->rm.slot, &hw.slot, 4, hipMemcpyHostToDevice, st));
    WIS_HIP_CHECK(hipMemcpyAsync(m->rm.lslot, &hw.slot, 4, hipMemcpyHostToDevice, st));
    WIS_HIP_CHECK(hipMemcpyAsync(m->bs.cum, &hw.cum, 4, hipMemcpyHostToDevice, st));
    WIS_RET(reseed_tick(m, steps));
  }
  return WIS_OK;
}

struct StepGraph {
  const GenCtx& g;
  ~StepGraph() { g.m->sa_nb = 8; }

  int nb_for(int passes_done) const {
    static const bool sa_short = !(getenv("WIS_SA_NB") && atoi(getenv("WIS_SA_NB")) == 0);
    const int len = g.P + passes_done;
    return !sa_short ? 8 : (len <= 16 ? 2 : (len <= 32 ? 4 : 8));
  }
  int one_step() const {
    WIS_RET(dec_forward(g.m, g.B * g.beam, g.beam, g.B, true, g.beam, 1));
    return sampling_tail(g, {g.beam, 1, 0}, TAIL_TAPS);
  }
  int graph_for(int nb, hipGraphExec_t* out) const {
    wis_model* m = g.m; const SampleCfg& sc = g.sc;
    GraphKey key; memset(&key, 0, sizeof(key));
    key.B = g.B; key.beam = g.beam; key.P = g.P; key.max_new = g.max_new; key.fixed_new = sc.fixed_new; key.suppress_blank = sc.suppress_blank;
    key.suppress_default = g.o->suppress_default; key.early_exit = sc.allow_early_exit; key.lp = sc.length_penalty; key.patience = g.patience; key.spin = m->spin_now ? 1 : 0;
    key.sa_nb = nb;
    key.timestamps = g.ts ? 1 : 0; key.max_init = g.ts ? g.ts_max_init : 0;
    key.rep_pen = g.rep_pen == 1.f ? 0.f : g.rep_pen; key.rep_ngram = g.rep_ngram;
    auto it = m->graphs.find(key);
    if (it != m->graphs.end()) { *out = it->second; return WIS_OK; }
    hipGraph_t graph = nullptr; hipGraphExec_t ge = nullptr;
    WIS_HIP_CHECK(hipStreamBeginCapture(g.st, hipStreamCaptureModeThreadLocal));
    int rc = one_step();
    hipError_t e = hipStreamEndCapture(g.st, &graph);
    if (rc) { if (graph) hipGraphDestroy(graph); return rc; }
    if (e != hipSuccess) { set_error("graph capture failed: %s", hipGetErrorString(e)); return WIS_E_HIP; }
    e = hipGraphInstantiate(&ge, graph, nullptr, nullptr, 0);
    hipGraphDestroy(graph);
    if (e != hipSuccess) { set_error("graph instantiate failed: %s", hipGetErrorString(e)); return WIS_E_HIP; }
    m->graphs[key] = ge;
    *out = ge;
    return WIS_OK;
  }
  int launch_pass(int passes_done) const {
    wis_model* m = g.m;
    m->sa_nb = nb_for(passes_done);
    if (!m->use_graph) return one_step();
    hipGraphExec_t ge = nullptr;
    WIS_RET(graph_for(m->sa_nb, &ge));
    WIS_HIP_CHECK(hipGraphLaunch(ge, g.st));
    return WIS_OK;
  }
};

struct LoopResult {
  int steps;
  int needed = 0;
  bool gave_up = false;
  bool from_host = false;
  float decode_ms_dev = -1.f;
};
static void unpack_progress(const wis_model* m, int* st_, int* dn_, int* gu_) {
  const unsigned long long r = __atomic_load_n(&m->h_prog[HP_REC], __ATOMIC_ACQUIRE);
  if ((r >> 48) != (unsigned long long)m->gen) { *st_ = 0; *dn_ = 0; *gu_ = 0; return; }
  *st_ = (int)((r >> 32) & 0xFFFFu); *gu_ = (int)((r >> 16) & 0xFFFFu); *dn_ = (int)(r & 0xFFFFu);
}
static int check_terminated(const GenCtx& g, LoopResult* lr, int dn_, int gu_) {
  lr->gave_up = gu_ != 0;
  if (!lr->gave_up && dn_ < g.B) { set_error("decode did not terminate within %d steps (done %d of %d)", lr->steps, dn_, g.B); return WIS_E_STATE; }
  return WIS_OK;
}

static int run_burst(const GenCtx& g, const StepGraph& sg, int limit, LoopResult* lr) {
  wis_model* m = g.m;
  for (; lr->steps < limit; ++lr->steps) WIS_RET(sg.launch_pass(lr->steps));
  WIS_HIP_CHECK(hipEventRecord(m->ev[5], g.st));
  WIS_HIP_CHECK(hipStreamSynchronize(g.st));
  int st_, dn_, gu_; unpack_progress(m, &st_, &dn_, &gu_);
  WIS_RET(check_terminated(g, lr, dn_, gu_));
  lr->needed = lr->steps;
  return WIS_OK;
}

static int run_paced(const GenCtx& g, const StepGraph& sg, int limit, int base_done, LoopResult* lr) {
  wis_model* m = g.m; const int B = g.B;
  int& steps = lr->steps;
  const auto t_dec0 = std::chrono::steady_clock::now();
  const int depth = g.o->queue_depth > 0 ? g.o->queue_depth : 2;
  auto t_last = std::chrono::steady_clock::now();
  int seen = -1, st_ = 0, dn_ = 0, gu_ = 0;
  static const bool trace = getenv("WIS_EOT_TRACE") != nullptr;
  struct Tr { int step; unsigned long long dev; double host_us; int launched; };
  std::vector<Tr> tr;
  const auto t_loop = std::chrono::steady_clock::now();
  for (unsigned spins = 0;; ++spins) {
    unpack_progress(m, &st_, &dn_, &gu_);
    if (st_ < base_done) st_ = base_done;
    if (dn_ >= B || gu_) break;
    if (st_ >= limit) break;
    if (steps < limit && steps - st_ < depth) {
      const auto tl0 = std::chrono::steady_clock::now();
      WIS_RET(sg.launch_pass(steps));
      ++steps;
      if (trace) tr.push_back({-steps, 0ull, std::chrono::duration<double, std::micro>(std::chrono::steady_clock::now() - tl0).count(), steps});
      continue;
    }
    if (st_ != seen) {
      seen = st_; t_last = std::chrono::steady_clock::now(); spins = 0;
      if (trace) tr.push_back({st_, m->h_prog[HP_STAMP], std::chrono::duration<double, std::micro>(t_last - t_loop).count(), steps});
    }
    else if ((spins & 1023u) == 1023u) {
      const double idle = std::chrono::duration<double>(std::chrono::steady_clock::now() - t_last).count();
      if (idle > 30.0) { set_error("decode made no progress for 30 s (step %d of %d enqueued)", st_, steps); return WIS_E_HIP; }
      if (idle > 200e-6) { struct timespec ts = {0, 20000}; nanosleep(&ts, nullptr); }
    }
    cpu_relax();
  }
  if (trace) {
    unsigned long long prev_dev = 0;
    for (size_t i = 0; i < tr.size(); ++i) {
      if (tr[i].step < 0) { fprintf(stderr, "[eot-trace]   launch of step %d took the host %.1f us\n", -tr[i].step, tr[i].host_us); continue; }
      fprintf(stderr, "[eot-trace] step %d seen by the host at %.1f us (device clock +%.1f us since the previous record), %d steps enqueued\n", tr[i].step, tr[i].host_us,
              prev_dev ? (double)(tr[i].dev - prev_dev) * 0.01 : 0.0, tr[i].launched);
      prev_dev = tr[i].dev;
    }
    fprintf(stderr, "[eot-trace] done seen at %.1f us: %d of %d utterances, %d steps enqueued\n", std::chrono::duration<double, std::micro>(std::chrono::steady_clock::now() - t_loop).count(), dn_, B, steps);
  }
  WIS_RET(check_terminated(g, lr, dn_, gu_));
  if (!lr->gave_up) {
    lr->from_host = true;
    lr->needed = (int)m->h_prog[HP_DONE_STEP];
    const unsigned long long s0 = m->h_prog[HP_STAMP0], s1 = m->h_prog[HP_DONE_STAMP];
    lr->decode_ms_dev = s1 > s0 ? (float)((double)(s1 - s0) * 1e-5) : 0.f;
    if (g.drafting) lr->decode_ms_dev = std::chrono::duration<float, std::milli>(std::chrono::steady_clock::now() - t_dec0).count();
  }
  return WIS_OK;
}

static void results_from_verification(const GenCtx& g, const Seed& sd, int32_t* out_ids, int32_t* out_len, float* out_score) {
  float sfin = sd.spec_cum;
  if (g.sc.length_penalty != 0.f) sfin /= powf((float)sd.spec_len, g.sc.length_penalty);
  out_len[0] = sd.spec_len;
  for (int t = 0; t < g.max_new; ++t) out_ids[t] = t < sd.spec_len ? sd.spec_gen[t] : 0;
  if (out_score) out_score[0] = sfin;
}
static int results_from_record(const GenCtx& g, int32_t* out_ids, int32_t* out_len, float* out_score) {
  const wis_model* m = g.m; const int max_new = g.max_new;
  const int* hl = hp_out_len(m->h_prog); const float* hs = hp_out_score(m->h_prog); const int* hi = hp_out_ids(m->h_prog);
  for (int b = 0; b < g.B; ++b) {
    int n = hl[b];
    if (n < 0 || n > max_new) { set_error("decode result of utterance %d has length %d outside [0, %d]", b, n, max_new); return WIS_E_STATE; }
    out_len[b] = n;
    for (int t = 0; t < max_new; ++t) out_ids[(size_t)b * max_new + t] = t < n ? hi[(size_t)b * max_new + t] : 0;
    if (out_score) out_score[b] = hs[b];
  }
  return WIS_OK;
}
static int results_from_device(wis_model* m, int B, int max_new, int32_t* out_ids, int32_t* out_len, float* out_score) {
  hipStream_t st = m->st;
  std::vector<int32_t> ids((size_t)B * MAX_STEPS);
  std::vector<float> sc_h(B);
  WIS_HIP_CHECK(hipMemcpyAsync(ids.data(), m->bs.out_ids, (size_t)B * MAX_STEPS * 4, hipMemcpyDeviceToHost, st));
  WIS_HIP_CHECK(hipMemcpyAsync(out_len, m->bs.out_len, (size_t)B * 4, hipMemcpyDeviceToHost, st));
  WIS_HIP_CHECK(hipMemcpyAsync(sc_h.data(), m->bs.out_score, (size_t)B * 4, hipMemcpyDeviceToHost, st));
  WIS_HIP_CHECK(hipStreamSynchronize(st));
  for (int b = 0; b < B; ++b) {
    if (out_len[b] > max_new) out_len[b] = max_new;
    for (int t = 0; t < max_new; ++t) out_ids[(size_t)b * max_new + t] = t < out_len[b] ? ids[(size_t)b * max_new + t] : 0;
    if (out_score) out_score[b] = sc_h[b];
  }
  return WIS_OK;
}
// ... 109 lines not shown
```

### willow-inference-server_amd/csrc/kernels.hpp

```cpp
#pragma once
#include "common.hpp"

namespace wis {

struct GemmP {
  const f16* A; int64_t a_bs; int a_rs; int a_rpb;
  const f16* W;
  int M, N, K;
  int klen;
  int n_span = 0, n_period = 0, n_phase = 0;
};
static inline GemmP gemm_plain(const f16* A, int lda, const f16* W, int M, int N, int K) {
  GemmP p; p.A = A; p.a_bs = 0; p.a_rs = lda; p.a_rpb = 0x7fffffff; p.W = W; p.M = M; p.N = N; p.K = K; p.klen = 0; return p;
}
int launch_layernorm(hipStream_t st, const float* x, const float* gamma, const float* beta, f16* y, int M, int d);
int launch_gemm_generic(hipStream_t st, const GemmP& p, const float* bias, const float* resid, void* C, int flags);
int launch_gemm_splitk_resid(hipStream_t st, const GemmP& p, int splits, float* scratch, const float* bias, const float* resid, float* X,
                             const float* ln_gamma = nullptr, const float* ln_beta = nullptr, f16* Y = nullptr);
int launch_gemm_conv1(hipStream_t st, const GemmP& p, const float* bias, f16* C, int T);
int launch_gemm_conv2(hipStream_t st, const GemmP& p, const float* bias, const float* pos, float* X, int T);
int launch_gemm_qkv(hipStream_t st, const GemmP& p, const float* bias, f16* qk, f16* vt, int d, int T, int Tpad, int H);
int launch_gemm_crosskv(hipStream_t st, const GemmP& p, const float* bias, f16* kx, f16* vt, int d, int T, int Tpad, int H, int64_t kx_lstride, int64_t vt_lstride);
int launch_enc_attention(hipStream_t st, const f16* qk, const f16* vt, f16* out, int B, int T, int Tpad, int H, float* part = nullptr, unsigned* counters = nullptr,
                         size_t part_cap = 0);
int launch_enc_attention_form(hipStream_t st, const f16* qk, const f16* vt, f16* out, int B, int T, int Tpad, int H, float* part, unsigned* counters,
                              bool lazy, bool split);
size_t enc_attention_part_floats(int B, int T, int H);
bool enc_attn_lazy();
void launch_scale_q_log2e(hipStream_t st, f16* qk, int64_t rows, int d);

constexpr int MAX_ROWS = 96;
constexpr int MAX_R = 8;
constexpr int MAX_CAND = 2 * MAX_R;
constexpr int MAX_HYP = 3 * MAX_R;

struct RowMeta {
  int* tok;
  int* pos;
  int* slot;
  int* lslot;
};

enum { GV_GELU = 1, GV_RESID = 2, GV_OUT_F32 = 4, GV_LN = 8, GV_QKV = 16,
       GV_LN16 = 64 };
struct GemvP {
  const void* x;
  const float* gamma; const float* beta;
  const float* csum;
  const f16* Wp; const float* bias;
  const float* wscale;
  void* y;
  int M, N, K, flags;
  float* q; f16* kc; f16* vc; const int* slot; const int* pos; int d; int ctx;
  unsigned long long* prof;
  int rows;
  const void* x2; int xsplit;
  f16* y16;
  int xmb;
  const float* stat_in;
  float* stat_out;
  f16* y_xf;
  int ymb;
  int ksplit; float* kpart; unsigned* kcnt;
  int mb0, mbi;
  int wks, wk0;
};
int launch_gemv(hipStream_t st, const GemvP& p);
int launch_gemv_dual(hipStream_t st, const GemvP& pa, const GemvP& pb);
int launch_gemv_frag(hipStream_t st, const GemvP& p);
int launch_gemv_frag3(hipStream_t st, const GemvP* p, int n);
__host__ __device__ static inline size_t xf_index(int m, int k, int MB) {
  return ((size_t)((k >> 5) * MB + (m >> 4)) * 64 + (m & 15) + 16 * ((k >> 3) & 3)) * 8 + (k & 7);
}
constexpr size_t xf_elems(int K, int MB) { return (size_t)(K / 32) * MB * 64 * 8; }
int launch_xf_pack(hipStream_t st, const void* x, int x_f16, f16* xf, float* stat, int M, int K, int MB);
int launch_dec_embed_xf(hipStream_t st, const f16* emb, const f16* pos_emb, const int* tok, const int* pos, float* x, f16* xf, float* stat, int M, int d, int MB);
int launch_fold_ln(hipStream_t st, f16* W, const float* gamma, const float* beta, float* bias, float* csum, int N, int K, int n_scale, float qscale);
int launch_csum8(hipStream_t st, const f16* W, const float* scale, float* csum, int N, int K, int n_scale, float qscale);
int launch_pack_gemv8(hipStream_t st, const f16* W, unsigned char* Wp, float* scale, int N, int Npad, int K, int n_scale, float qscale);
int launch_pack_gemv(hipStream_t st, const f16* W, f16* Wp, int N, int Npad, int K, int n_scale, float scale, int rows = 16);
int launch_pack_gemv_nc8(hipStream_t st, const f16* W, f16* Wp, int N, int Npad, int K);
bool gemv_nc8_shape(int M, int N, int K);
int gemv_rows_for(int N, int K);

int launch_dec_embed(hipStream_t st, const f16* emb, const f16* pos_emb, const int* tok, const int* pos, float* x, int M, int d, f16* xh = nullptr);
struct SelfAttnP {
  const float* q = nullptr; const f16* kc = nullptr; const f16* vc = nullptr; const int* pos = nullptr; f16* out = nullptr;
  int M = 0, H = 0, d = 0, ctx = 0, rpu = 0, sstride = 0, rmul = 0;
  unsigned long long* prof = nullptr; int out_mb = 0; const int* anc = nullptr; int w0 = 0, aw = 0;
  const int* base = nullptr;
  int nb = 8;
};
int launch_dec_self_attn(hipStream_t st, const SelfAttnP& p);
constexpr int CA_SPIN_MAX_BH = 192;
struct CrossAttnP {
  const float* q = nullptr; const f16* kx = nullptr; const f16* vt = nullptr; f16* out = nullptr; float* part = nullptr; unsigned* counters = nullptr;
  int B = 0, R = 0, H = 0, d = 0, T = 0, Tpad = 0, chunks = 0;
  unsigned long long* prof = nullptr; int out_mb = 0;
  const float* xres = nullptr; const float* qcs = nullptr; const float* qb = nullptr;
  unsigned long long* gran = nullptr; unsigned* epoch = nullptr;
  const float* q2 = nullptr; int xres_is_stat = 0;
  int kv_shared = 0;
};
int launch_dec_cross_attn(hipStream_t st, const CrossAttnP& p);

struct SampleCfg {
  int n_vocab, n_vocab_pad, eot, beam, n_cand, max_new, fixed_new, suppress_blank, greedy;
  float length_penalty; int max_hyp; int allow_early_exit; int max_candidates;
  int early_exit_hyps;
};
#ifndef WIS_EARLY_EXIT_NUM_HYPOTHESES
#define WIS_EARLY_EXIT_NUM_HYPOTHESES 1
#endif
constexpr int STAT_SUB = 64;
int launch_logit_stats(hipStream_t st, const float* logits, const float* bias_all, const float* bias_begin, const int* step_u,
                       float* st_max, float* st_sum, float* st_val, int* st_idx, int B, const SampleCfg& cfg,
                       int lr_b, int lr_j, int lr_off, unsigned long long* prof = nullptr,
                       const int* rowmap = nullptr,
                       const int* ts_desc = nullptr);
constexpr int TS_DESC_INTS = 8;
struct BeamState;
int launch_ts_rules(hipStream_t st, const float* logits, const float* bias_all, const float* bias_begin, const BeamState& bs, int B,
                    const SampleCfg& cfg, int no_ts, int max_init, int lr_b, int lr_j, int lr_off, int* ts_desc);
int launch_rep_rules(hipStream_t st, float* logits, const BeamState& bs, int B, const SampleCfg& cfg, float penalty, int ngram, int lr_b, int lr_j, int lr_off);
int launch_no_speech(hipStream_t st, const float* logits, int ld, int B, int rs, int r0, int V, int ns, float* out);
struct BeamState {
  int* step_u;
  int* done;
  int* n_hyp;
  float* cum;
  int* alive;
  int* parent;
  float* hyp_score;
  int* hyp_len;
  int* hyp_tok;
  int* all_done;
  int* out_ids; int* out_len; float* out_score;
  unsigned* tick;
  const unsigned* giveup;
  unsigned long long* host;
  int* traj;
};
enum { HP_REC = 0,
       HP_STAMP0 = 1,
       HP_STAMP = 2,
       HP_DONE_STEP = 3,
       HP_DONE_STAMP = 4,
       HP_WORDS = 8,
       HP_MAXB = MAX_ROWS };
constexpr size_t HP_BYTES = HP_WORDS * 8 + (size_t)HP_MAXB * 8 + (size_t)HP_MAXB * 256 * 4;
__host__ __device__ inline int* hp_out_len(unsigned long long* hp) { return reinterpret_cast<int*>(hp + HP_WORDS); }
__host__ __device__ inline float* hp_out_score(unsigned long long* hp) { return reinterpret_cast<float*>(hp + HP_WORDS) + HP_MAXB; }
__host__ __device__ inline int* hp_out_ids(unsigned long long* hp) { return reinterpret_cast<int*>(hp + HP_WORDS) + 2 * HP_MAXB; }
int launch_kv_reorder(hipStream_t st, f16* kc, f16* vc, size_t layer_stride, int L, const BeamState& bs, int B, int beam, int P, int ctx, int d);
int launch_beam_step(hipStream_t st, const float* st_max, const float* st_sum, const float* st_val, const int* st_idx,
                     const BeamState& bs, const RowMeta& rm, int B, int P, int ctx, const SampleCfg& cfg, unsigned long long* prof = nullptr);
constexpr int DRAFT_VS_INTS = 32 + MAX_R * 32, DRAFT_VS_PERM = 8, DRAFT_VS_BASE = 16;
int launch_draft_match(hipStream_t st, const BeamState& bs, const int* draft, int n_draft, int beam, int* vstate, int book);
int launch_kv_gather(hipStream_t st, f16* kc, f16* vc, size_t layer_stride, int L, const int* vstate, const int* done, int beam, int w0, int ctx, int d);
int launch_greedy_pick(hipStream_t st, const float* st_max, const float* st_sum, const float* st_val, const int* st_idx, int rows, const SampleCfg& cfg, int* tok_out, float* lp_out);
int launch_lang_probs(hipStream_t st, const float* logits, int ld, const int* lang_ids, int n_lang, float* probs, int B);

}
```

### willow-inference-server_amd/csrc/model.hip

```cpp
#include <math.h>
#include <stdlib.h>
#include <string.h>
#include <time.h>
#include <algorithm>
#include <array>
#include <atomic>
#include <chrono>
#include <map>
#include <mutex>
#include <memory>
#include <string>
#include <vector>

#include "common.hpp"
#include "kernels.hpp"

using namespace wis;

namespace wis {

__global__ void convert_kernel(const void* __restrict__ src, int src_f16, void* __restrict__ dst, int dst_f16,
                               int64_t rows, int64_t cols, int64_t dst_ld, int64_t n_scale, float scale) {
  const int64_t total = rows * cols;
  for (int64_t i = (int64_t)blockIdx.x * blockDim.x + threadIdx.x; i < total; i += (int64_t)gridDim.x * blockDim.x) {
// ... 636 lines not shown
struct DeferredClaim { hipEvent_t ev; int n; };
static std::mutex g_spin_mu;
static std::vector<DeferredClaim> g_spin_deferred[64];
static void spin_collect(int device) {
  std::lock_guard<std::mutex> lk(g_spin_mu);
  auto& v = g_spin_deferred[device & 63];
  for (size_t i = 0; i < v.size();) {
    if (hipEventQuery(v[i].ev) != hipErrorNotReady) { g_spin_bh[device & 63].fetch_sub(v[i].n, std::memory_order_relaxed); v[i] = v.back(); v.pop_back(); }
    else ++i;
  }
}
struct SpinClaim {
  wis_model* m; int n = 0;
  SpinClaim(wis_model* mm, int B) : m(mm) {
    static const bool env_share = getenv("WIS_CA_SPIN_SHARED") != nullptr;
    m->spin_now = false;
    spin_collect(m->device);
    if (m->spin_off) return;
    if (env_share) { m->spin_now = true; return; }
    const int need = B * m->cfg.n_heads;
    std::atomic<int>& a = g_spin_bh[m->device & 63];
    int cur = a.load(std::memory_order_relaxed);
    while (cur + need <= CA_SPIN_MAX_BH)
      if (a.compare_exchange_weak(cur, cur + need, std::memory_order_relaxed)) { n = need; m->spin_now = true; return; }
  }
  ~SpinClaim() { if (n) g_spin_bh[m->device & 63].fetch_sub(n, std::memory_order_relaxed); }
  void defer(hipStream_t st) {
    if (!n) return;
    if (hipEventRecord(m->ev[6], st) != hipSuccess) return;
    std::lock_guard<std::mutex> lk(g_spin_mu);
    auto& v = g_spin_deferred[m->device & 63];
    for (auto& d : v) if (d.ev == m->ev[6]) { d.n += n; n = 0; return; }
    v.push_back({m->ev[6], n}); n = 0;
  }
  SpinClaim(const SpinClaim&) = delete;
  SpinClaim& operator=(const SpinClaim&) = delete;
};
static int spin_gave_up(wis_model* m, bool* gave_up) {
  int* h = &m->h_pin->giveup;
  WIS_HIP_CHECK(hipMemcpyAsync(h, m->ca_epoch, 4, hipMemcpyDeviceToHost, m->st));
  WIS_HIP_CHECK(hipStreamSynchronize(m->st));
  *gave_up = *h != 0;
  if (*gave_up) {
    WIS_HIP_CHECK(hipMemsetAsync(m->ca_epoch, 0, 4, m->st));
    m->spin_off = true; ++m->handoff_retries;
    fprintf(stderr, "[wis_hip] device %d: decoder cross-attention granule hand-off timed out; this handle uses the ticket hand-off from now on, the call is repeated\n", m->device);
  }
  return WIS_OK;
}

struct TreeWin { const int* anc; int w0, aw; const int* base = nullptr; };
int align_capture_q(wis_model* m, int l, int M);

static GemvP gemv_small(const DecProj& p, const void* x, void* y, int M, int flags) {
  GemvP g; memset(&g, 0, sizeof(g));
  g.x = x; g.csum = p.csum; g.Wp = p.Wp; g.wscale = p.scale; g.bias = p.bias; g.y = y; g.M = M; g.N = p.N; g.K = p.K; g.flags = flags; g.rows = p.rows;
  if (p.Wp8 && !(flags & ~(GV_RESID | GV_OUT_F32 | GV_GELU)) && gemv_nc8_shape(M, p.N, p.K)) { g.Wp = p.Wp8; g.rows = 8; }
  return g;
}
static GemvP gemv_frag(const DecProj& p, const void* xf, int M, int flags) {
  GemvP g; memset(&g, 0, sizeof(g));
  g.x = xf; g.csum = p.csum; g.Wp = p.Wp; g.wscale = p.scale; g.bias = p.bias; g.M = M; g.N = p.N; g.K = p.K; g.flags = flags; g.xmb = cdiv(M, 16); g.rows = 16;
  return g;
}
static void out_cq_dual(const DecLayerW& w, const f16* a, const f16* xh, float* x1, float* stat, float* q, int M, GemvP* ga, GemvP* gb) {
  const int d = w.out.K;
  memset(ga, 0, sizeof(*ga));
  ga->x = a; ga->Wp = w.out.Wp; ga->bias = w.out.bias; ga->y = x1; ga->M = M; ga->N = d; ga->K = d; ga->flags = GV_RESID; ga->stat_out = stat;
  memset(gb, 0, sizeof(*gb));
  gb->x = xh; gb->x2 = a; gb->xsplit = d; gb->Wp = w.cqo.Wp; gb->bias = w.cqo.bias; gb->y = q; gb->M = M; gb->N = d; gb->K = w.cqo.K; gb->flags = GV_OUT_F32;
}
static void out_cq_frag3(const DecLayerW& w, const f16* af, const f16* xf, float* x1, float* stat, float* q, float* q2, int M, GemvP g3[3]) {
  const int d = w.out.K;
  g3[0] = gemv_frag(w.out, af, M, GV_RESID);
  g3[0].wscale = nullptr; g3[0].y = x1; g3[0].ymb = g3[0].xmb; g3[0].stat_out = stat;
  g3[1] = gemv_frag(w.cqo, xf, M, GV_OUT_F32);
  g3[1].K = d; g3[1].y = q; g3[1].wks = w.cqo.K / 32; g3[1].wk0 = 0;
  g3[2] = gemv_frag(w.cqo, af, M, GV_OUT_F32);
  g3[2].K = d; g3[2].bias = nullptr; g3[2].y = q2; g3[2].wks = w.cqo.K / 32; g3[2].wk0 = d / 32;
}

static int dec_forward_frag(wis_model* m, int M, int R, int B, bool want_logits, int sstride, int rmul, int chunks, const TreeWin* tw = nullptr) {
  const wis_config_t& c = m->cfg; hipStream_t st = m->st;
  const int d = c.d_model, H = c.n_heads, T = c.n_audio_ctx, ctx = c.n_text_ctx, MB = cdiv(M, 16);
  if (tw && (M % 16 != 0 || R != 16 || B != M / 16)) { set_error("dec_forward_frag: a tree window takes whole groups of 16 rows"); return WIS_E_ARG; }
  WIS_RET(launch_dec_embed_xf(st, m->emb, m->dec_pos, m->rm.tok, m->rm.pos, m->dx, m->dxf, m->dstat, M, d, MB));
  static const bool no_frag_fold = getenv("WIS_NO_FRAG_FOLD") != nullptr;
  const bool fold = m->cq_fold && !no_frag_fold && R <= 8;
  SelfAttnP sa;
  sa.q = m->dq; sa.pos = m->rm.pos; sa.out = m->daoxf; sa.M = M; sa.H = H; sa.d = d; sa.ctx = ctx; sa.rpu = R; sa.sstride = sstride; sa.rmul = rmul; sa.out_mb = MB; sa.nb = m->sa_nb;
  if (tw) { sa.anc = tw->anc; sa.w0 = tw->w0; sa.aw = tw->aw; sa.base = tw->base; }
  CrossAttnP ca;
  ca.q = m->dq; ca.out = m->daoxf; ca.part = m->part; ca.counters = m->counters; ca.B = B; ca.R = R; ca.H = H; ca.d = d; ca.T = T; ca.Tpad = m->Tpad; ca.chunks = chunks; ca.out_mb = MB;
  ca.epoch = m->ca_epoch;
  for (int l = 0; l < c.n_dec_layers; ++l) {
    const DecLayerW& w = m->dec[l];
    unsigned long long* pr = (m->prof_on && l == 0) ? m->d_prof : nullptr;
    GemvP g = gemv_frag(w.qkv, m->dxf, M, GV_LN | GV_QKV);
    g.stat_in = m->dstat; g.q = m->dq; g.kc = m->kc[l]; g.vc = m->vc[l]; g.slot = m->rm.slot; g.pos = m->rm.pos; g.d = d; g.ctx = ctx;
    g.prof = pr;
    WIS_RET(launch_gemv_frag(st, g));
    sa.kc = m->kc[l]; sa.vc = m->vc[l];
    WIS_RET(launch_dec_self_attn(st, sa));
    if (fold) {
      if (m->al.capture) { set_error("dec_forward_frag: an alignment pass needs the un-folded route (more than 8 rows per utterance)"); return WIS_E_STATE; }
      GemvP g3[3];
      out_cq_frag3(w, m->daoxf, m->dxf, m->dx, m->dstat, m->dq, m->dq2, M, g3);
      g3[0].prof = pr ? pr + 32 : nullptr;
      WIS_RET(launch_gemv_frag3(st, g3, 3));
      CrossAttnP cf = ca;
      cf.kx = m->kx[l]; cf.vt = m->vx[l]; cf.prof = pr ? pr + 64 : nullptr; cf.xres = m->dstat; cf.qcs = w.cq.csum; cf.qb = w.cq.bias;
      cf.gran = m->spin_now ? m->ca_gran : nullptr; cf.q2 = m->dq2; cf.xres_is_stat = 1;
      WIS_RET(launch_dec_cross_attn(st, cf));
    } else {
    g = gemv_frag(w.out, m->daoxf, M, GV_RESID);
    g.y = m->dx; g.y_xf = m->dxf; g.ymb = MB; g.stat_out = m->dstat;
    WIS_RET(launch_gemv_frag(st, g));
    g = gemv_frag(w.cq, m->dxf, M, GV_LN | GV_OUT_F32);
    g.stat_in = m->dstat; g.y = m->dq;
    WIS_RET(launch_gemv_frag(st, g));
    const size_t ku = (size_t)m->al.kv_ub0 * H * T * 64, vu = (size_t)m->al.kv_ub0 * H * 64 * m->Tpad;
    CrossAttnP cp = ca;
    cp.kx = m->kx[l] + ku; cp.vt = m->vx[l] + vu; cp.gran = (m->spin_now && !tw) ? m->ca_gran : nullptr; cp.kv_shared = tw ? 1 : 0;
    WIS_RET(launch_dec_cross_attn(st, cp));
    if (m->al.capture) WIS_RET(align_capture_q(m, l, M));
    }
    g = gemv_frag(w.cout, m->daoxf, M, GV_RESID);
    g.y = m->dx; g.y_xf = m->dxf; g.ymb = MB; g.stat_out = m->dstat; g.prof = pr ? pr + 80 : nullptr;
    WIS_RET(launch_gemv_frag(st, g));
    g = gemv_frag(w.f1, m->dxf, M, GV_LN | GV_GELU);
    g.stat_in = m->dstat; g.y = m->dhxf; g.ymb = MB; g.prof = pr ? pr + 96 : nullptr;
    WIS_RET(launch_gemv_frag(st, g));
    g = gemv_frag(w.f2, m->dhxf, M, GV_RESID);
    g.y = m->dx; g.y_xf = m->dxf; g.ymb = MB; g.stat_out = m->dstat; g.prof = pr ? pr + 112 : nullptr;
    if (m->gf_ksplit > 1 && (4 * d / 32) % (4 * m->gf_ksplit) == 0) { g.ksplit = m->gf_ksplit; g.kpart = m->gf_part; g.kcnt = m->gf_cnt; }
    WIS_RET(launch_gemv_frag(st, g));
  }
  if (want_logits) {
    GemvP g = gemv_frag(m->proj, m->dxf, M, GV_LN | GV_OUT_F32);
    g.stat_in = m->dstat; g.y = m->logits;
    WIS_RET(launch_gemv_frag(st, g));
  }
  return WIS_OK;
}

struct StepRoute { bool frag, fold, ln16; };
static StepRoute small_route(const wis_model* m, int M) {
  static const bool ln_f16 = [] { const char* e = getenv("WIS_B1_LN"); return e && !strcmp(e, "f16"); }();
  const int d = m->cfg.d_model;
  const bool frag = M > 8, ln_ok = !frag && m->cq_fold && d % 64 == 0 && M * (d / 8) <= 13 * 256;
  return {frag, m->cq_fold, ln_ok && ln_f16 && d <= 2048};
}

int dec_forward(wis_model* m, int M, int R, int B, bool want_logits, int sstride, int rmul, const TreeWin* tw = nullptr) {
  const wis_config_t& c = m->cfg; hipStream_t st = m->st;
  const int d = c.d_model, H = c.n_heads, T = c.n_audio_ctx, ctx = c.n_text_ctx;
  static const int env_chunks = getenv("WIS_CROSS_CHUNKS") ? atoi(getenv("WIS_CROSS_CHUNKS")) : 0;
  const int chunks = env_chunks ? env_chunks : 6;
  const StepRoute rt = small_route(m, M);
  if (tw || rt.frag) return dec_forward_frag(m, M, R, B, want_logits, sstride, rmul, chunks, tw);
  if (m->al.capture) { set_error("wis_align needs the batched-row decoder route (more than 8 rows per pass)"); return WIS_E_STATE; }
  const bool fold = rt.fold, ln16 = rt.ln16;
  const int ln = ln16 ? GV_LN16 : GV_LN;
  auto ln_x = [&](const f16* x16) { return ln16 ? (const void*)x16 : (const void*)m->dx; };
  WIS_RET(launch_dec_embed(st, m->emb, m->dec_pos, m->rm.tok, m->rm.pos, m->dx, M, d, fold ? m->dxh : nullptr));
  SelfAttnP sa;
  sa.q = m->dq; sa.pos = m->rm.pos; sa.out = m->dao; sa.M = M; sa.H = H; sa.d = d; sa.ctx = ctx; sa.rpu = R; sa.sstride = sstride; sa.rmul = rmul; sa.nb = m->sa_nb;
  CrossAttnP ca;
  ca.q = m->dq; ca.out = m->dao; ca.part = m->part; ca.counters = m->counters; ca.B = B; ca.R = R; ca.H = H; ca.d = d; ca.T = T; ca.Tpad = m->Tpad; ca.chunks = chunks;
  ca.gran = m->spin_now ? m->ca_gran : nullptr; ca.epoch = m->ca_epoch;
  for (int l = 0; l < c.n_dec_layers; ++l) {
    const DecLayerW& w = m->dec[l];
    unsigned long long* pr = (m->prof_on && (l == 0 || m->prof_all)) ? m->d_prof + (size_t)l * 8 * 16 : nullptr;
    GemvP g = gemv_small(w.qkv, ln_x(m->dxh), nullptr, M, ln | GV_QKV);
    g.q = m->dq; g.kc = m->kc[l]; g.vc = m->vc[l]; g.slot = m->rm.slot; g.pos = m->rm.pos; g.d = d; g.ctx = ctx;
    g.prof = pr;
    WIS_RET(launch_gemv(st, g));
    sa.kc = m->kc[l]; sa.vc = m->vc[l]; sa.prof = pr ? pr + 16 : nullptr;
    WIS_RET(launch_dec_self_attn(st, sa));
    ca.kx = m->kx[l]; ca.vt = m->vx[l]; ca.prof = pr ? pr + 64 : nullptr;
    if (fold) {
      GemvP ga, gb;
      out_cq_dual(w, m->dao, m->dxh, m->dx, m->dstat, m->dq, M, &ga, &gb);
      ga.prof = pr ? pr + 32 : nullptr;
      WIS_RET(launch_gemv_dual(st, ga, gb));
      CrossAttnP cf = ca;
      cf.xres = m->dstat; cf.qcs = w.cq.csum; cf.qb = w.cq.bias; cf.xres_is_stat = 1;
      WIS_RET(launch_dec_cross_attn(st, cf));
    } else {
    g = gemv_small(w.out, m->dao, m->dx, M, GV_RESID);
    g.prof = pr ? pr + 32 : nullptr;
    WIS_RET(launch_gemv(st, g));
    g = gemv_small(w.cq, m->dx, m->dq, M, GV_LN | GV_OUT_F32);
    g.prof = pr ? pr + 48 : nullptr;
    WIS_RET(launch_gemv(st, g));
    WIS_RET(launch_dec_cross_attn(st, ca));
    }
    g = gemv_small(w.cout, m->dao, m->dx, M, GV_RESID);
    g.prof = pr ? pr + 80 : nullptr;
    if (ln16) g.y16 = m->dln;
    WIS_RET(launch_gemv(st, g));
    g = gemv_small(w.f1, ln_x(m->dln), m->dh, M, ln | GV_GELU);
    g.prof = pr ? pr + 96 : nullptr;
    WIS_RET(launch_gemv(st, g));
    g = gemv_small(w.f2, m->dh, m->dx, M, GV_RESID);
    g.prof = pr ? pr + 112 : nullptr;
    g.y16 = fold ? m->dxh : nullptr;
    WIS_RET(launch_gemv(st, g));
  }
  if (want_logits) WIS_RET(launch_gemv(st, gemv_small(m->proj, ln_x(m->dxh), m->logits, M, ln | GV_OUT_F32)));
  return WIS_OK;
}

static int init_beam_state(wis_model* m, int B, int beam) {
  hipStream_t st = m->st;
  const int Mrows = B * beam;
  float* cum = m->h_pin->beam_cum;
  for (int r = 0; r < Mrows; ++r) cum[r] = (r % beam == 0) ? 0.f : -INFINITY;
  unsigned* tk = m->h_pin->beam_tick;
  m->gen = (m->gen % 0xFFFFu) + 1u;
  tk[0] = 0; tk[1] = m->gen; tk[2] = 0; tk[3] = 0;
  WIS_HIP_CHECK(hipMemcpyAsync(m->bs.cum, cum, (size_t)Mrows * 4, hipMemcpyHostToDevice, st));
  WIS_HIP_CHECK(hipMemcpyAsync(m->bs.tick, tk, 16, hipMemcpyHostToDevice, st));
  WIS_HIP_CHECK(hipMemsetAsync(m->bs.step_u, 0, (size_t)B * 4, st));
  WIS_HIP_CHECK(hipMemsetAsync(m->bs.done, 0, (size_t)B * 4, st));
  WIS_HIP_CHECK(hipMemsetAsync(m->bs.n_hyp, 0, (size_t)B * 4, st));
  WIS_HIP_CHECK(hipMemsetAsync(m->bs.all_done, 0, 16, st));
  WIS_HIP_CHECK(hipMemsetAsync(m->bs.out_len, 0, (size_t)B * 4, st));
  return WIS_OK;
}
static SampleCfg make_sample_cfg(const wis_model* m, const wis_gen_opts_t* o, int beam, int max_new, float* patience_out) {
  const wis_config_t& c = m->cfg;
  SampleCfg sc; memset(&sc, 0, sizeof(sc));
  sc.n_vocab = c.n_vocab; sc.n_vocab_pad = m->n_vocab_pad; sc.eot = c.eot; sc.beam = beam; sc.n_cand = 2 * beam; sc.max_new = max_new;
  sc.fixed_new = o->fixed_new_tokens; sc.suppress_blank = o->suppress_blank; sc.greedy = beam == 1;
  sc.length_penalty = o->length_penalty; sc.max_hyp = MAX_HYP;
  const float patience = o->patience > 0.f ? o->patience : 1.f;
  sc.max_candidates = (int)lroundf((float)beam * patience); if (sc.max_candidates < 1) sc.max_candidates = 1;
  sc.allow_early_exit = (patience == 1.f && o->length_penalty == 0.f) ? 1 : 0;
  sc.early_exit_hyps = WIS_EARLY_EXIT_NUM_HYPOTHESES ? 1 : sc.max_candidates;
  *patience_out = patience;
  return sc;
}

static int check_patience(int beam, float patience) {
  const float p = patience > 0.f ? patience : 1.f;
  const long want = lroundf((float)beam * p);
  if (want > MAX_HYP - beam + 1) {
    set_error("patience %.3g at beam_size %d needs %ld finished hypotheses; the engine holds %d (patience <= %.3g at this beam)", (double)p, beam, want, MAX_HYP - beam + 1,
              (double)(MAX_HYP - beam + 1) / (double)beam);
    return WIS_E_ARG;
  }
  return WIS_OK;
}

int upload_rows(wis_model* m, const std::vector<int>& tok, const std::vector<int>& pos, const std::vector<int>& slot, const std::vector<int>& lslot, bool wait = true, RowStage* stage = nullptr) {
  const size_t n = tok.size();
  RowStage* h = stage ? stage : &m->h_pin->rows;
  memcpy(h->tok, tok.data(), n * 4); memcpy(h->pos, pos.data(), n * 4); memcpy(h->slot, slot.data(), n * 4); memcpy(h->lslot, lslot.data(), n * 4);
  WIS_HIP_CHECK(hipMemcpyAsync(m->rm.tok, h->tok, n * 4, hipMemcpyHostToDevice, m->st));
  WIS_HIP_CHECK(hipMemcpyAsync(m->rm.pos, h->pos, n * 4, hipMemcpyHostToDevice, m->st));
  WIS_HIP_CHECK(hipMemcpyAsync(m->rm.slot, h->slot, n * 4, hipMemcpyHostToDevice, m->st));
  WIS_HIP_CHECK(hipMemcpyAsync(m->rm.lslot, h->lslot, n * 4, hipMemcpyHostToDevice, m->st));
  if (wait) WIS_HIP_CHECK(hipStreamSynchronize(m->st));
  return WIS_OK;
}

int check_batch(wis_model* m, int B, int beam) {
  if (B < 1 || B > m->cfg.max_batch) { set_error("batch %d outside [1, max_batch=%d]", B, m->cfg.max_batch); return WIS_E_STATE; }
  if (beam < 1 || beam > m->cfg.max_beam || beam > MAX_R) { set_error("beam_size %d outside [1, %d]", beam, m->cfg.max_beam < MAX_R ? m->cfg.max_beam : MAX_R); return WIS_E_STATE; }
  if (B * beam > MAX_ROWS) { set_error("B*beam = %d exceeds %d decoder rows per device batch", B * beam, MAX_ROWS); return WIS_E_STATE; }
  return WIS_OK;
}

static std::atomic<int> g_active_calls[64];
struct BusyGuard {
  wis_model* m; bool ok;
  explicit BusyGuard(wis_model* mm) : m(mm), ok(!mm->busy.test_and_set(std::memory_order_acquire)) { if (ok) g_active_calls[m->device & 63].fetch_add(1, std::memory_order_relaxed); }
  ~BusyGuard() { if (ok) { g_active_calls[m->device & 63].fetch_sub(1, std::memory_order_relaxed); m->busy.clear(std::memory_order_release); } }
};
#define WIS_ENTER(m, what)                                                                                      \
  BusyGuard _busy(m);                                                                                           \
  if (!_busy.ok) { set_error("%s: another call is running on this handle (one call at a time per replica)", what); return WIS_E_STATE; }

}

extern "C" {

int wis_version(void) { return WIS_ABI_VERSION; }
const char* wis_last_error(void) { return get_error(); }
int wis_device_count(void) { int n = 0; if (hipGetDeviceCount(&n) != hipSuccess) return 0; return n; }
int wis_supported_compute_types(int device, char* out, size_t cap) {
  (void)device;
  const char* s = "float16,float32,int8_float16";
  if (!out || cap < strlen(s) + 1) { set_error("buffer too small"); return WIS_E_ARG; }
  strcpy(out, s); return WIS_OK;
}

int wis_model_create(const wis_config_t* cfg, const void* arena, size_t arena_bytes, int arena_on_device,
                     const wis_tensor_t* tensors, int n_tensors, int device, wis_model_t** out) {
  if (!cfg || !arena || !tensors || !out || n_tensors <= 0) { set_error("wis_model_create: bad argument"); return WIS_E_ARG; }
  if (cfg->d_model % 128 || cfg->d_model != cfg->n_heads * 64 || cfg->d_model > 2048 || !mel_bins_supported(cfg->n_mels) || cfg->n_enc_layers < 1 || cfg->n_dec_layers < 1 || cfg->n_audio_ctx != 1500 ||
      cfg->n_text_ctx > 512 || cfg->max_batch < 1 || cfg->max_beam < 1 || cfg->max_beam > MAX_R || cfg->n_vocab < 1024) {
    set_error("wis_model_create: unsupported config (d_model %% 128, head_dim 64, n_mels 80 or 128, n_audio_ctx 1500, max_beam <= %d)", MAX_R);
    return WIS_E_UNSUPPORTED;
  }
  DeviceCtx* ctx; WIS_RET(get_ctx(device, &ctx));
  wis_model* m = new wis_model();
  m->cfg = *cfg; m->device = device; m->ctx = ctx;
  m->w8 = cfg->decoder_weight_bits == 8;
  m->cq_fold = !m->w8 && getenv("WIS_NO_CQFOLD") == nullptr;
  m->use_graph = getenv("WIS_NO_GRAPH") == nullptr;
  memset(&m->timing, 0, sizeof(m->timing));
  int rc = WIS_OK;
  void* d_arena = nullptr;
  do {
    if (hipStreamCreateWithFlags(&m->st, hipStreamNonBlocking) != hipSuccess) { set_error("stream create failed"); rc = WIS_E_HIP; break; }
    const char* base = reinterpret_cast<const char*>(arena);
    if (!arena_on_device) {
      if (hipMalloc(&d_arena, arena_bytes) != hipSuccess) { set_error("hipMalloc(arena %zu) failed", arena_bytes); rc = WIS_E_NOMEM; break; }
      if (hipMemcpy(d_arena, arena, arena_bytes, hipMemcpyHostToDevice) != hipSuccess) { set_error("arena upload failed"); rc = WIS_E_HIP; break; }
      base = reinterpret_cast<const char*>(d_arena);
    }
    Loader L{tensors, n_tensors, base, arena_bytes};
    if ((rc = load_weights(m, L))) break;
    {
      std::vector<float> ba(m->n_vocab_pad, 0.f), bb(m->n_vocab_pad, 0.f);
      for (int i = 0; i < cfg->n_suppress; ++i) if (cfg->suppress_ids[i] >= 0 && cfg->suppress_ids[i] < cfg->n_vocab) ba[cfg->suppress_ids[i]] = -INFINITY;
      for (int i = 0; i < cfg->n_suppress_begin; ++i) if (cfg->suppress_ids_begin[i] >= 0 && cfg->suppress_ids_begin[i] < cfg->n_vocab) bb[cfg->suppress_ids_begin[i]] = -INFINITY;
      if ((rc = dalloc(m, &m->bias_all, ba.size())) || (rc = dalloc(m, &m->bias_begin, bb.size()))) break;
      hipMemcpy(m->bias_all, ba.data(), ba.size() * 4, hipMemcpyHostToDevice);
      hipMemcpy(m->bias_begin, bb.data(), bb.size() * 4, hipMemcpyHostToDevice);
      if ((rc = dalloc(m, &m->d_lang_ids, (size_t)(cfg->n_lang > 0 ? cfg->n_lang : 1)))) break;
      if (cfg->n_lang > 0) hipMemcpy(m->d_lang_ids, cfg->lang_ids, (size_t)cfg->n_lang * 4, hipMemcpyHostToDevice);
    }
    m->cfg.suppress_ids = nullptr; m->cfg.suppress_ids_begin = nullptr; m->cfg.lang_ids = nullptr;
    m->wslabs = std::make_shared<WeightSlabs>();
    m->wslabs->device = device; m->wslabs->slabs.swap(m->allocs); m->wslabs->bytes = m->bytes;
    m->slab_cur = nullptr; m->slab_left = 0;
    if ((rc = alloc_buffers(m))) break;
    if (hipStreamSynchronize(m->st) != hipSuccess) { set_error("model init failed"); rc = WIS_E_HIP; break; }
  } while (0);
  if (d_arena) hipFree(d_arena);
  if (rc) { wis_model_destroy(m); return rc; }
  *out = m;
  return WIS_OK;
}

void wis_model_destroy(wis_model_t* m) {
  if (!m) return;
  hipSetDevice(m->device);
  if (m->st) hipStreamSynchronize(m->st);
  spin_collect(m->device);
  for (auto& kv : m->graphs) hipGraphExecDestroy(kv.second);
  for (void* p : m->allocs) hipFree(p);
  if (m->h_pin) hipHostFree(m->h_pin);
  if (m->h_prog) hipHostFree(m->h_prog);
  for (int i = 0; i < 8; ++i) if (m->ev[i]) hipEventDestroy(m->ev[i]);
  for (hipEvent_t e : m->al.ev) if (e) hipEventDestroy(e);
  if (m->st_enc) { hipStreamSynchronize(m->st_enc); hipStreamDestroy(m->st_enc); }
  if (m->ev_enc) hipEventDestroy(m->ev_enc);
  if (m->ev_ckv) hipEventDestroy(m->ev_ckv);
  if (m->st) hipStreamDestroy(m->st);
  delete m;
// ... 160 lines not shown
```

### willow-inference-server_amd/csrc/taps.hip

```cpp
namespace {
struct Tap {
  const char* const name;
  hipStream_t st = nullptr;
  int rc;
  Tap(int device, const char* who) : name(who) {
    DeviceCtx* c = nullptr;
    if ((rc = get_ctx(device, &c)) != WIS_OK) return;
    lock = std::unique_lock<std::mutex>(ctx_op_mutex(c));
    st = ctx_stream(c);
  }
  Tap(const Tap&) = delete;
  Tap& operator=(const Tap&) = delete;
  template <class T> int get(T** p, size_t n_elems, bool zeroed = false) {
    const size_t bytes = n_elems * sizeof(T) ? n_elems * sizeof(T) : 16;
    void* q = nullptr;
    if (hipMalloc(&q, bytes) != hipSuccess) { (void)hipGetLastError(); set_error("%s: out of device memory", name); return WIS_E_NOMEM; }
    scratch.push_back(q); *p = reinterpret_cast<T*>(q);
    if (zeroed) hipMemsetAsync(q, 0, bytes, st);
    return WIS_OK;
  }
  int finish(int launch_rc) {
    const hipError_t e0 = hipGetLastError(), e = hipStreamSynchronize(st);
    synced = true;
    if (launch_rc) return launch_rc;
// ... 406 lines not shown
  Tap t(device, "wis_op_gemv_qkv"); WIS_RET(t.rc);
  if (!x || !gamma || !beta || !W || !bias || !slot || !pos || !q || !kc || !vc || M < 1 || M > MAX_ROWS || d < 128 || d % 128 || ctx < 1) { set_error("wis_op_gemv_qkv: bad argument"); return WIS_E_ARG; }
  hipStream_t st = t.st;
  const int N = 3 * d, MB = cdiv(M, 16);
  const float qs = 0.125f;
  f16 *wp = nullptr, *wtmp = nullptr, *xf = nullptr; float *b2 = nullptr, *cs = nullptr, *stt = nullptr;
  WIS_RET(t.get(&wp, (size_t)N * d)); WIS_RET(t.get(&wtmp, (size_t)N * d)); WIS_RET(t.get(&b2, (size_t)N)); WIS_RET(t.get(&cs, (size_t)N, true));
  if (M > 8) { WIS_RET(t.get(&xf, xf_elems(d, MB), true)); WIS_RET(t.get(&stt, (size_t)M * (d / 16) * 2)); }
  hipMemcpyAsync(wtmp, W, (size_t)N * d * 2, hipMemcpyDeviceToDevice, st);
  hipLaunchKernelGGL(convert_kernel, dim3(blocks_for(N)), dim3(256), 0, st, bias, 0, b2, 0, (int64_t)N, (int64_t)1, (int64_t)1, (int64_t)d, qs);
  const DecProj qkv{wp, nullptr, b2, cs, N, d, gemv_rows_for(N, d)};
  WIS_RET(prep_projection(st, wtmp, N, N, d, d, qs, gamma, beta, b2, cs, wp, nullptr, qkv.rows));
  GemvP g;
  if (M <= 8) g = gemv_small(qkv, x, nullptr, M, GV_LN | GV_QKV);
  else {
    WIS_RET(launch_xf_pack(st, x, 0, xf, stt, M, d, MB));
    g = gemv_frag(qkv, xf, M, GV_LN | GV_QKV);
    g.stat_in = stt;
  }
  g.q = q; g.kc = reinterpret_cast<f16*>(kc); g.vc = reinterpret_cast<f16*>(vc); g.slot = slot; g.pos = pos; g.d = d; g.ctx = ctx;
  return t.finish(M <= 8 ? launch_gemv(st, g) : launch_gemv_frag(st, g));
}

int wis_op_gemv_out_cq(int device, const void* a, const float* x0, const void* Wo, const float* bo, const void* Wq, const float* bq, const float* gamma, const float* beta,
                       float* x1, float* stat, float* q, float* q2, float* qcs, float* qb, int M, int d, int force_frag) {
  Tap t(device, "wis_op_gemv_out_cq"); WIS_RET(t.rc);
  const bool frag = M > 8 || force_frag;
  if (!a || !x0 || !Wo || !bo || !Wq || !bq || !gamma || !beta || !x1 || !stat || !q || !qcs || !qb || (frag && !q2) || M < 1 || M > MAX_ROWS || d < 128 || d % 128) {
    set_error("wis_op_gemv_out_cq: bad argument"); return WIS_E_ARG; }
  hipStream_t st = t.st;
  const int MB = cdiv(M, 16);
  const float qs = 0.125f;
  f16 *wtmp = nullptr, *fcat = nullptr, *fwot = nullptr, *fwqo = nullptr, *p_cqo = nullptr, *p_out = nullptr, *xh = nullptr, *xf = nullptr, *af = nullptr; float* b_cqo = nullptr;
  WIS_RET(t.get(&wtmp, (size_t)d * d)); WIS_RET(t.get(&fcat, (size_t)2 * d * d)); WIS_RET(t.get(&fwot, (size_t)d * d)); WIS_RET(t.get(&fwqo, (size_t)d * d));
  WIS_RET(t.get(&p_cqo, (size_t)2 * d * d)); WIS_RET(t.get(&p_out, (size_t)d * d)); WIS_RET(t.get(&b_cqo, (size_t)d));
  if (frag) { WIS_RET(t.get(&xf, xf_elems(d, MB), true)); WIS_RET(t.get(&af, xf_elems(d, MB), true)); }
  else WIS_RET(t.get(&xh, (size_t)M * d));
  hipMemcpyAsync(wtmp, Wq, (size_t)d * d * 2, hipMemcpyDeviceToDevice, st);
  hipLaunchKernelGGL(convert_kernel, dim3(blocks_for(d)), dim3(256), 0, st, bq, 0, qb, 0, (int64_t)d, (int64_t)1, (int64_t)1, (int64_t)d, qs);
  hipMemsetAsync(qcs, 0, (size_t)d * 4, st);
  DecLayerW w{};
  w.out = DecProj{p_out, nullptr, bo, nullptr, d, d, gemv_rows_for(d, d)};
  w.cqo = DecProj{p_cqo, nullptr, b_cqo, nullptr, d, 2 * d, 16};
  WIS_RET(prep_projection(st, wtmp, d, d, d, d, qs, gamma, beta, qb, qcs, nullptr, nullptr, 16));
  WIS_RET(launch_pack_gemv(st, reinterpret_cast<const f16*>(Wo), p_out, d, d, d, 0, 1.f, w.out.rows));
  WIS_RET(build_cq_fold(st, wtmp, Wo, 1, bo, d, qs, fcat, fwot, fwqo, p_cqo, b_cqo));
  hipMemcpyAsync(x1, x0, (size_t)M * d * 4, hipMemcpyDeviceToDevice, st);
  if (!frag) {
    hipLaunchKernelGGL(convert_kernel, dim3(blocks_for((int64_t)M * d)), dim3(256), 0, st, x0, 0, xh, 1, (int64_t)M, (int64_t)d, (int64_t)d, (int64_t)0, 1.f);
    GemvP ga, gb;
    out_cq_dual(w, reinterpret_cast<const f16*>(a), xh, x1, stat, q, M, &ga, &gb);
    return t.finish(launch_gemv_dual(st, ga, gb));
  }
  WIS_RET(launch_xf_pack(st, x0, 0, xf, nullptr, M, d, MB));
  WIS_RET(launch_xf_pack(st, a, 1, af, nullptr, M, d, MB));
  GemvP g3[3];
  out_cq_frag3(w, af, xf, x1, stat, q, q2, M, g3);
  return t.finish(launch_gemv_frag3(st, g3, 3));
}

int wis_op_mel_to_image(int device, const float* mel, void* img_f16, int B, int n_mels) {
  Tap t(device, "wis_op_mel_to_image"); WIS_RET(t.rc);
  if (!mel || !img_f16 || B < 1) { set_error("wis_op_mel_to_image: bad argument"); return WIS_E_ARG; }
  return t.finish(launch_mel_to_image(t.st, mel, reinterpret_cast<f16*>(img_f16), B, n_mels));
}
int wis_op_enc_conv(int device, int which, const void* img_f16, const void* W, int w_is_f16, const float* bias, const float* pos, void* out,
                    int B, int T, int Cin, int N) {
  Tap t(device, "wis_op_enc_conv"); WIS_RET(t.rc);
  if (!img_f16 || !W || !bias || !out || B < 1 || T < 1 || N < 128 || (which != 1 && which != 2) || (which == 2 && !pos) || (int64_t)B * (2 * (int64_t)T + 2) > 0x7fffffff) {
    set_error("wis_op_enc_conv: bad argument"); return WIS_E_ARG; }
  if (which == 1 ? !mel_bins_supported(Cin) : (Cin < 64 || Cin % 64)) { set_error("wis_op_enc_conv: conv%d with %d input channels", which, Cin); return WIS_E_UNSUPPORTED; }
  f16* wp = nullptr;
  WIS_RET(t.get(&wp, (size_t)N * (which == 1 ? conv1_k(Cin) : 3 * Cin)));
  if (which == 1) {
    pack_conv1_w(t.st, W, w_is_f16, wp, N, Cin);
    return t.finish(launch_gemm_conv1(t.st, conv1_gemm(reinterpret_cast<const f16*>(img_f16), wp, B, T, Cin, N), bias, reinterpret_cast<f16*>(out), T));
  }
  pack_conv2_w(t.st, W, w_is_f16, wp, N, Cin);
  return t.finish(launch_gemm_conv2(t.st, conv2_gemm(reinterpret_cast<const f16*>(img_f16), wp, B, T, Cin, N), bias, pos, reinterpret_cast<float*>(out), T));
}
int wis_op_enc_qkv(int device, const void* xn_f16, const void* W_f16, const float* bias, void* qk_f16, void* vt_f16, int B, int T, int H) {
  Tap t(device, "wis_op_enc_qkv"); WIS_RET(t.rc);
  if (!xn_f16 || !W_f16 || !bias || !qk_f16 || !vt_f16 || B < 1 || T < 1 || H < 1 || (int64_t)B * T > 0x7fffffff / (3 * 64 * (int64_t)H)) { set_error("wis_op_enc_qkv: bad argument"); return WIS_E_ARG; }
  if (T % 4) { set_error("wis_op_enc_qkv: T = %d (the transposed V tiles store 4 consecutive keys of one utterance: T %% 4 == 0)", T); return WIS_E_ARG; }
  const int d = 64 * H;
  return t.finish(launch_gemm_qkv(t.st, gemm_plain(reinterpret_cast<const f16*>(xn_f16), d, reinterpret_cast<const f16*>(W_f16), B * T, 3 * d, d), bias,
                                  reinterpret_cast<f16*>(qk_f16), reinterpret_cast<f16*>(vt_f16), d, T, cdiv(T, 64) * 64, H));
}
int wis_op_enc_crosskv(int device, const void* mem_f16, const void* W_f16, const float* bias, void* kx_f16, void* vt_f16, int B, int T, int H, int L,
                       int64_t kx_lstride, int64_t vt_lstride) {
  Tap t(device, "wis_op_enc_crosskv"); WIS_RET(t.rc);
  if (!mem_f16 || !W_f16 || !bias || !kx_f16 || !vt_f16 || B < 1 || T < 1 || H < 1 || L < 1 || (int64_t)L * 2 * 64 * H > 0x7fffffff || (int64_t)B * T > 0x7fffffff / (64 * (int64_t)H)) {
    set_error("wis_op_enc_crosskv: bad argument"); return WIS_E_ARG; }
  if (T % 4) { set_error("wis_op_enc_crosskv: T = %d (the transposed V tiles store 4 consecutive keys of one utterance: T %% 4 == 0)", T); return WIS_E_ARG; }
  const int d = 64 * H, Tpad = cdiv(T, 64) * 64;
  if (kx_lstride < (int64_t)B * T * d || vt_lstride < (int64_t)B * d * Tpad || kx_lstride % 8 || vt_lstride % 8) {
    set_error("wis_op_enc_crosskv: layer strides must be multiples of 8 elements and at least the layer's image"); return WIS_E_ARG; }
  return t.finish(launch_gemm_crosskv(t.st, gemm_plain(reinterpret_cast<const f16*>(mem_f16), d, reinterpret_cast<const f16*>(W_f16), B * T, L * 2 * d, d), bias,
                                      reinterpret_cast<f16*>(kx_f16), reinterpret_cast<f16*>(vt_f16), d, T, Tpad, H, kx_lstride, vt_lstride));
}
int wis_op_gemm_splitk_ln(int device, const void* A_f16, const void* W_f16, const float* bias, float* X, const float* gamma, const float* beta, void* Y_f16,
                          int M, int N, int K, int splits) {
  Tap t(device, "wis_op_gemm_splitk_ln"); WIS_RET(t.rc);
  if (!A_f16 || !W_f16 || !bias || !X || !gamma || !beta || !Y_f16 || M < 1 || N < 128 || K < 64 || splits < 0 || splits > 16 || (int64_t)M * N > 0x7fffffff) {
    set_error("wis_op_gemm_splitk_ln: bad argument"); return WIS_E_ARG; }
  if (!splits) splits = enc_splitk(N, M);
  if (!splits) { set_error("wis_op_gemm_splitk_ln: the encoder does not split K at M = %d, N = %d", M, N); return WIS_E_UNSUPPORTED; }
  float* scratch = nullptr;
  WIS_RET(t.get(&scratch, (size_t)splits * M * N));
  return t.finish(launch_gemm_splitk_resid(t.st, gemm_plain(reinterpret_cast<const f16*>(A_f16), K, reinterpret_cast<const f16*>(W_f16), M, N, K), splits, scratch, bias, X, X,
                                           gamma, beta, reinterpret_cast<f16*>(Y_f16)));
}

int wis_op_kv_reorder(int device, void* kc_f16, void* vc_f16, int64_t layer_stride_elems, int L, const int32_t* parent, const int32_t* step_u, const int32_t* done,
                      int B, int beam, int P, int ctx, int d) {
  Tap t(device, "wis_op_kv_reorder"); WIS_RET(t.rc);
  if (!kc_f16 || !vc_f16 || !parent || !step_u || !done || L < 1 || B < 1 || beam < 1 || P < 1 || ctx < 1 || d < 8 || d % 8 || layer_stride_elems < (int64_t)B * beam * ctx * d || layer_stride_elems % 8) {
    set_error("wis_op_kv_reorder: bad argument"); return WIS_E_ARG; }
  BeamState bs; memset(&bs, 0, sizeof(bs));
  bs.parent = const_cast<int*>(parent); bs.step_u = const_cast<int*>(step_u); bs.done = const_cast<int*>(done);
  return t.finish(launch_kv_reorder(t.st, reinterpret_cast<f16*>(kc_f16), reinterpret_cast<f16*>(vc_f16), (size_t)layer_stride_elems, L, bs, B, beam, P, ctx, d));
}
int wis_op_kv_gather(int device, void* kc_f16, void* vc_f16, int64_t layer_stride_elems, int L, const int32_t* vstate, const int32_t* done, int beam, int w0, int ctx, int d) {
  Tap t(device, "wis_op_kv_gather"); WIS_RET(t.rc);
  if (!kc_f16 || !vc_f16 || !vstate || !done || L < 1 || beam < 1 || beam > MAX_R || w0 < 0 || w0 >= ctx || d < 8 || d % 8 || layer_stride_elems < (int64_t)beam * ctx * d || layer_stride_elems % 8) {
    set_error("wis_op_kv_gather: bad argument"); return WIS_E_ARG; }
  return t.finish(launch_kv_gather(t.st, reinterpret_cast<f16*>(kc_f16), reinterpret_cast<f16*>(vc_f16), (size_t)layer_stride_elems, L, vstate, done, beam, w0, ctx, d));
}
int wis_op_no_speech(int device, const float* logits, int ld, int B, int rs, int r0, int V, int ns, float* out) {
  Tap t(device, "wis_op_no_speech"); WIS_RET(t.rc);
  if (!logits || !out || B < 1 || rs < 1 || r0 < 0 || r0 >= rs || V < 1 || ld < V) { set_error("wis_op_no_speech: bad argument"); return WIS_E_ARG; }
  return t.finish(launch_no_speech(t.st, logits, ld, B, rs, r0, V, ns, out));
}
int wis_op_lang_probs(int device, const float* logits, int ld, const int32_t* lang_ids, int n_lang, float* probs, int B) {
  Tap t(device, "wis_op_lang_probs"); WIS_RET(t.rc);
  if (!logits || !lang_ids || !probs || B < 1 || n_lang < 1 || ld < 1) { set_error("wis_op_lang_probs: bad argument"); return WIS_E_ARG; }
  return t.finish(launch_lang_probs(t.st, logits, ld, lang_ids, n_lang, probs, B));
}
int wis_op_greedy_rows(int device, const float* logits, int n_vocab, int n_vocab_pad, int eot, const float* bias_all, const float* bias_begin, const int32_t* step_u,
                       int B, int beam, int lr_b, int lr_j, int lr_off, const int32_t* rowmap, int32_t* tok_out, float* lp_out) {
  Tap t(device, "wis_op_greedy_rows"); WIS_RET(t.rc);
  if (!logits || !bias_begin || !step_u || !tok_out || !lp_out || B < 1 || beam < 1 || beam > MAX_R || n_vocab < STAT_SUB || n_vocab_pad < n_vocab || eot < 0 || eot >= n_vocab ||
      lr_b < 0 || lr_j < 0 || lr_off < 0) { set_error("wis_op_greedy_rows: bad argument"); return WIS_E_ARG; }
  const int rows = B * beam;
  SampleCfg sc; memset(&sc, 0, sizeof(sc));
  sc.n_vocab = n_vocab; sc.n_vocab_pad = n_vocab_pad; sc.eot = eot; sc.beam = beam; sc.n_cand = 2; sc.suppress_blank = 1; sc.greedy = 1;
  float *smax = nullptr, *ssum = nullptr, *sval = nullptr; int* sidx = nullptr;
  WIS_RET(t.get(&smax, (size_t)rows * STAT_SUB)); WIS_RET(t.get(&ssum, (size_t)rows * STAT_SUB));
  WIS_RET(t.get(&sval, (size_t)rows * STAT_SUB * sc.n_cand)); WIS_RET(t.get(&sidx, (size_t)rows * STAT_SUB * sc.n_cand));
  WIS_RET(launch_logit_stats(t.st, logits, bias_all, bias_begin, step_u, smax, ssum, sval, sidx, B, sc, lr_b, lr_j, lr_off, nullptr, rowmap));
  return t.finish(launch_greedy_pick(t.st, smax, ssum, sval, sidx, rows, sc, tok_out, lp_out));
}

}
```

### willow-inference-server_amd/wis_hip/_lib.py

```python
import ctypes as C
import os

import numpy as np

_HERE = os.path.dirname(os.path.abspath(__file__))
LIB_PATH = os.environ.get("WIS_LIB_PATH") or os.path.join(os.path.dirname(_HERE), "lib", "libwis_hip.so")

WIS_OK = 0
WIS_IN_MEL_HOST, WIS_IN_MEL_DEV, WIS_IN_PCM_HOST, WIS_IN_PCM_DEV = 0, 1, 2, 3
WIS_DT_F32, WIS_DT_F16 = 0, 1
N_SAMPLES, N_FRAMES, N_MELS = 480000, 3000, 80


class WisError(RuntimeError):
    def __init__(self, code, msg):
        super().__init__(f"libwis_hip error {code}: {msg}")
        self.code = code


class Config(C.Structure):
    _fields_ = [(n, C.c_int32) for n in ("d_model", "n_heads", "n_enc_layers", "n_dec_layers", "n_vocab", "n_audio_ctx",
                                          "n_text_ctx", "n_mels", "max_batch", "max_beam", "eot", "sot", "no_timestamps",
                                          "no_speech")] + [
        ("suppress_ids", C.POINTER(C.c_int32)), ("n_suppress", C.c_int32),
        ("suppress_ids_begin", C.POINTER(C.c_int32)), ("n_suppress_begin", C.c_int32),
        ("lang_ids", C.POINTER(C.c_int32)), ("n_lang", C.c_int32), ("decoder_weight_bits", C.c_int32)]


class Tensor(C.Structure):
    _fields_ = [("name", C.c_char_p), ("dtype", C.c_int32), ("rank", C.c_int32), ("shape", C.c_int64 * 4), ("offset", C.c_uint64)]


class GenOpts(C.Structure):
    _fields_ = [("input_kind", C.c_int32), ("beam_size", C.c_int32), ("max_new_tokens", C.c_int32), ("length_penalty", C.c_float),
                ("patience", C.c_float), ("suppress_blank", C.c_int32), ("suppress_default", C.c_int32),
                ("fixed_new_tokens", C.c_int32), ("queue_depth", C.c_int32), ("timestamps", C.c_int32), ("max_initial_timestamp_index", C.c_int32),
                ("no_speech_prob", C.c_int32), ("repetition_penalty", C.c_float), ("no_repeat_ngram_size", C.c_int32)]


class Timing(C.Structure):
    _fields_ = [("logmel_ms", C.c_float), ("encoder_ms", C.c_float), ("crosskv_ms", C.c_float), ("prefill_ms", C.c_float),
                ("decode_ms", C.c_float), ("total_ms", C.c_float), ("decode_steps", C.c_int32), ("decode_steps_needed", C.c_int32)]

    def as_dict(self):
        return {n: getattr(self, n) for n, _ in self._fields_}


class SvConfig(C.Structure):
    _fields_ = [("conv_dim", C.c_int32), ("n_conv_layers", C.c_int32), ("conv_kernel", C.c_int32 * 8), ("conv_stride", C.c_int32 * 8),
                ("hidden_size", C.c_int32), ("n_heads", C.c_int32), ("n_layers", C.c_int32), ("intermediate_size", C.c_int32),
                ("num_conv_pos_embeddings", C.c_int32), ("num_conv_pos_embedding_groups", C.c_int32), ("num_buckets", C.c_int32),
                ("max_bucket_distance", C.c_int32), ("n_tdnn", C.c_int32), ("tdnn_dim", C.c_int32 * 8), ("tdnn_kernel", C.c_int32 * 8),
                ("tdnn_dilation", C.c_int32 * 8), ("xvector_output_dim", C.c_int32), ("max_samples", C.c_int64)]


_vp, _i, _sz, _i64 = C.c_void_p, C.c_int, C.c_size_t, C.c_int64
_fp = C.POINTER(C.c_float)
SYMBOLS = [
    ("wis_version", _i, []),
    ("wis_last_error", C.c_char_p, []),
    ("wis_device_count", _i, []),
    ("wis_supported_compute_types", _i, [_i, C.c_char_p, _sz]),
    ("wis_audio_decode", _i, [_vp, _sz, C.POINTER(_fp), C.POINTER(_i64), C.POINTER(_i), C.POINTER(_i)]),
    ("wis_audio_free", None, [_fp]),
    ("wis_logmel", _i, [_i, _vp, _i64, C.POINTER(_i64), _i, _i, _vp, _i]),
    ("wis_melstream_create", _i, [_i, C.POINTER(_vp)]),
    ("wis_logmel_n", _i, [_i, _i, _vp, _i64, C.POINTER(_i64), _i, _i, _vp, _i]),
    ("wis_melstream_create_n", _i, [_i, _i, C.POINTER(_vp)]),
    ("wis_melstream_reset", _i, [_vp]),
    ("wis_melstream_feed", _i, [_vp, _vp, _i64]),
    ("wis_melstream_finish", _i, [_vp, _vp, C.POINTER(_vp)]),
    ("wis_melstream_samples", _i64, [_vp]),
    ("wis_melstream_tiles_done", _i, [_vp]),
    ("wis_melstream_destroy", None, [_vp]),
    ("wis_model_create", _i, [C.POINTER(Config), _vp, _sz, _i, C.POINTER(Tensor), _i, _i, C.POINTER(_vp)]),
    ("wis_model_destroy", None, [_vp]),
    ("wis_model_device_bytes", _sz, [_vp]),
    ("wis_model_clone", _i, [_vp, C.POINTER(_vp)]),
    ("wis_generate", _i, [_vp, _vp, _i, C.POINTER(C.c_int32), _i, C.POINTER(GenOpts), C.POINTER(C.c_int32), C.POINTER(C.c_int32), _fp]),
    ("wis_generate_draft", _i, [_vp, _vp, C.POINTER(C.c_int32), _i, C.POINTER(GenOpts), C.POINTER(C.c_int32), _i, C.POINTER(C.c_int32), C.POINTER(C.c_int32), _fp,
                                C.POINTER(C.c_int32)]),
    ("wis_generate_draft_beam", _i, [_vp, _vp, C.POINTER(C.c_int32), _i, C.POINTER(GenOpts), C.POINTER(C.c_int32), C.POINTER(C.c_int32), _i, C.POINTER(C.c_int32),
                                     C.POINTER(C.c_int32), _fp, C.POINTER(C.c_int32)]),
    ("wis_last_trajectory", _i, [_vp, _i, C.POINTER(C.c_int32), C.POINTER(C.c_int32), _i, C.POINTER(C.c_int32)]),
    ("wis_last_no_speech_prob", _i, [_vp, _i, _fp]),
    ("wis_detect_language", _i, [_vp, _vp, _i, _i, _fp]),
    ("wis_debug_encode", _i, [_vp, _vp, _i, _i, _fp]),
    ("wis_debug_logits", _i, [_vp, _vp, _i, _i, C.POINTER(C.c_int32), _i, _fp]),
    ("wis_debug_logits_rows", _i, [_vp, _vp, _i, _i, C.POINTER(C.c_int32), _i, _i, _fp]),
    ("wis_model_set_alignment_heads", _i, [_vp, C.POINTER(C.c_int32), _i]),
    ("wis_align", _i, [_vp, _vp, _i, _i, C.POINTER(C.c_int32), _i, C.POINTER(C.c_int32), C.POINTER(C.c_int32), C.POINTER(C.c_int32), _i,
                       C.POINTER(C.c_int32), C.POINTER(C.c_int32), C.POINTER(C.c_int32), _fp]),
    ("wis_debug_align_matrix", _i, [_vp, _vp, _i, _i, C.POINTER(C.c_int32), _i, C.POINTER(C.c_int32), C.POINTER(C.c_int32), C.POINTER(C.c_int32), _i, _fp]),
    ("wis_align_last_timing", _i, [_vp, _fp]),
    ("wis_op_dtw", _i, [_i, _vp, _i, _i, _vp, _vp, _vp]),
    ("wis_op_align_matrix", _i, [_i, _vp, _vp, _i, _i, _i, _i, _i, _vp]),
    ("wis_debug_tree_logits", _i, [_vp, _vp, _i, C.POINTER(C.c_int32), _i, _i, C.POINTER(C.c_int32), C.POINTER(C.c_int32), _i, _fp]),
    ("wis_debug_search", _i, [_vp, _vp, _i, _i, C.POINTER(GenOpts), C.POINTER(C.c_int32), C.POINTER(C.c_int32), _fp, C.POINTER(C.c_int32), C.POINTER(C.c_int32)]),
    ("wis_debug_handoff", _i, [_vp, _i, C.POINTER(_i), C.POINTER(_i)]),
    ("wis_last_timing", _i, [_vp, C.POINTER(Timing)]),
    ("wis_debug_phase_cycles", _i, [_vp, _i, _i, _i, C.POINTER(C.c_uint64)]),
    ("wis_debug_timeline", _i, [_vp, _i, _i, _i, _i, C.POINTER(C.c_uint64), _i]),
    ("wis_debug_sampling_cycles", _i, [_vp, C.POINTER(C.c_uint64)]),
    ("wis_bench_weight_stream", _i, [_vp, _i, _i, _fp, C.POINTER(_i), C.POINTER(C.c_double)]),
    ("wis_dev_alloc", _i, [_i, _sz, C.POINTER(_vp)]),
    ("wis_dev_free", _i, [_i, _vp]),
    ("wis_dev_h2d", _i, [_i, _vp, _vp, _sz]),
    ("wis_dev_d2h", _i, [_i, _vp, _vp, _sz]),
    ("wis_dev_sync", _i, [_i]),
    ("wis_dev_copy_peer", _i, [_i, _vp, _i, _vp, _sz]),
    ("wis_op_gemm", _i, [_i, _vp, _i, _vp, _vp, _vp, _vp, _i, _i, _i, _i]),
    ("wis_op_layernorm", _i, [_i, _vp, _vp, _vp, _vp, _i, _i]),
    ("wis_op_enc_attention", _i, [_i, _vp, _vp, _vp, _i, _i, _i, _i]),
    ("wis_op_enc_attention_ex", _i, [_i, _vp, _vp, _vp, _i, _i, _i, _i, _i]),
    ("wis_op_gemv", _i, [_i, _vp, _vp, _vp, _vp, _vp, _vp, _i, _i, _i, _i]),
    ("wis_op_gemv_cols", _i, [_i, _vp, _vp, _vp, _vp, _vp, _i, _i, _i, _i, _i]),
    ("wis_op_dec_self_attn", _i, [_i, _vp, _vp, _vp, _vp, _vp, _i, _i, _i, _i, _i, _i]),
    ("wis_op_dec_cross_attn", _i, [_i, _vp, _vp, _vp, _vp, _i, _i, _i, _i, _i]),
    ("wis_op_dec_cross_attn_folded", _i, [_i, _vp, _vp, _vp, _vp, _vp, _vp, _vp, _i, _i, _i, _i, _i]),
    ("wis_op_dec_cross_attn_stat", _i, [_i] + [_vp] * 8 + [_i] * 8),
    ("wis_op_dec_self_attn_ex", _i, [_i, _vp, _vp, _vp, _vp, _vp, _i, _i, _i, _i, _i, _i, _i, _i, _vp, _i, _i, _vp]),
    ("wis_op_gemv_qkv", _i, [_i] + [_vp] * 10 + [_i] * 3),
    ("wis_op_gemv_out_cq", _i, [_i] + [_vp] * 14 + [_i] * 3),
    ("wis_op_mel_to_image", _i, [_i, _vp, _vp, _i, _i]),
    ("wis_op_enc_conv", _i, [_i, _i, _vp, _vp, _i, _vp, _vp, _vp, _i, _i, _i, _i]),
    ("wis_op_enc_qkv", _i, [_i] + [_vp] * 5 + [_i] * 3),
    ("wis_op_enc_crosskv", _i, [_i] + [_vp] * 5 + [_i] * 4 + [_i64] * 2),
    ("wis_op_gemm_splitk_ln", _i, [_i] + [_vp] * 7 + [_i] * 4),
    ("wis_op_kv_reorder", _i, [_i, _vp, _vp, _i64, _i, _vp, _vp, _vp, _i, _i, _i, _i, _i]),
    ("wis_op_kv_gather", _i, [_i, _vp, _vp, _i64, _i, _vp, _vp, _i, _i, _i, _i]),
    ("wis_op_no_speech", _i, [_i, _vp, _i, _i, _i, _i, _i, _i, _vp]),
    ("wis_op_lang_probs", _i, [_i, _vp, _i, _vp, _i, _vp, _i]),
    ("wis_op_greedy_rows", _i, [_i, _vp, _i, _i, _i, _vp, _vp, _vp, _i, _i, _i, _i, _i, _vp, _vp, _vp]),
    ("wis_sv_create", _i, [C.POINTER(SvConfig), _vp, _sz, _i, C.POINTER(Tensor), _i, _i, C.POINTER(_vp)]),
    ("wis_sv_destroy", None, [_vp]),
    ("wis_sv_device_bytes", _sz, [_vp]),
    ("wis_sv_embed", _i, [_vp, _vp, _i64, _fp]),
    ("wis_sv_rel_buckets", _i, [_i, _i, _i, _i, C.POINTER(C.c_int32)]),
    ("wis_debug_sv_taps", _i, [_vp, _vp, _i64, _i, _i, _fp, _i64, C.POINTER(C.c_int32), C.POINTER(C.c_int32)]),
    ("wis_op_sv_conv0", _i, [_i, _vp, _i64, _vp, _vp, _vp, _vp]),
    ("wis_op_sv_posconv", _i, [_i, _vp, _vp, _vp, _vp, _i]),
    ("wis_op_sv_attention", _i, [_i, _vp, _vp, _vp, _vp, _vp, _vp, _i, _vp, _i]),
    ("wis_op_sv_layernorm", _i, [_i, _vp, _i, _vp, _vp, _vp, _vp, _vp, _vp, C.c_float, _i, _i, _i]),
    ("wis_op_sv_xvector_tail", _i, [_i, _vp, _i, _i, _i, _vp, _vp, _vp, _vp]),
]

_lib = None


def load():
    global _lib
    if _lib is not None:
        return _lib
    if not os.path.exists(LIB_PATH):
        raise WisError(-5, f"{LIB_PATH} is not built (run `python willow-inference-server_amd/build.py`); "
                           "there is no CPU fallback for the ASR path")
    lib = C.CDLL(LIB_PATH)
    for name, res, args in SYMBOLS:
        fn = getattr(lib, name)
        fn.restype = res
        fn.argtypes = args
    if lib.wis_version() != 1:
        raise WisError(-6, "ABI version mismatch")
    _lib = lib
    return lib


def check(rc):
    if rc != WIS_OK:
        raise WisError(rc, (load().wis_last_error() or b"").decode(errors="replace"))


def device_count():
    return load().wis_device_count()


def require_gpu():
    n = device_count()
    if n < 1:
        raise WisError(-5, "no HIP device visible: the wis_hip ASR path needs a gfx950 GPU (no CPU fallback)")
    return n


def ptr(a):
    assert a.flags["C_CONTIGUOUS"]
    return a.ctypes.data_as(C.c_void_p)


class DevBuf:

    def __init__(self, nbytes, device=0):
        self.device, self.nbytes = device, int(nbytes)
        p = C.c_void_p()
        check(load().wis_dev_alloc(device, self.nbytes, C.byref(p)))
        self.ptr = p

    @classmethod
    def from_numpy(cls, a, device=0):
        a = np.ascontiguousarray(a)
        b = cls(a.nbytes, device)
        check(load().wis_dev_h2d(device, b.ptr, ptr(a), a.nbytes))
        return b

    def to_numpy(self, dtype, shape):
        out = np.empty(shape, dtype=dtype)
        assert out.nbytes <= self.nbytes
        check(load().wis_dev_d2h(self.device, ptr(out), self.ptr, out.nbytes))
        return out

    def free(self):
        if self.ptr:
            load().wis_dev_free(self.device, self.ptr)
            self.ptr = None

    def __del__(self):
        try:
            self.free()
        except Exception:
            pass
```

Measured before the change: 151.3 x realtime.

## Fuse next-step token embedding into beam step and skip begin-bias after first step

The beam step kernel now writes the next decoder input rows (token embedding plus positional embedding, f32 and optional f16 copy) right after choosing tokens, so the following decoder forward skips its separate embed kernel launch. Loads for the embedding are issued before the alive/history bookkeeping to overlap latency. A specialized logit_stats variant for steps past the first drops the bias_begin loads. This adds work and register pressure to the single-block-per-batch beam step kernel, and it needs extra embed calls after the draft and tree paths reseed.

```diff
diff --git a/include/wis_hip.h b/include/wis_hip.h
--- a/include/wis_hip.h
+++ b/include/wis_hip.h
@@ -214,6 +214,9 @@
 int wis_op_lang_probs(int device, const float* logits, int ld, const int32_t* lang_ids, int n_lang, float* probs, int B);
 int wis_op_greedy_rows(int device, const float* logits, int n_vocab, int n_vocab_pad, int eot, const float* bias_all, const float* bias_begin,
                        const int32_t* step_u, int B, int beam, int lr_b, int lr_j, int lr_off, const int32_t* rowmap, int32_t* tok_out, float* lp_out);
+int wis_debug_tail_rows(wis_model_t* m, const float* logits, int n_steps, int B, int P, const wis_gen_opts_t* opts, int stats_form, const float* bias_begin,
+                        uint32_t fill_x, uint16_t fill_xh, int32_t* out_tok, int32_t* out_pos, int32_t* out_done, float* out_x, uint16_t* out_xh,
+                        float* out_st_max, float* out_st_sum, float* out_st_val, int32_t* out_st_idx);
 
 typedef struct wis_sv wis_sv_t;
 typedef struct {
diff --git a/willow-inference-server_amd/csrc/dec_kernels.hip b/willow-inference-server_amd/csrc/dec_kernels.hip
--- a/willow-inference-server_amd/csrc/dec_kernels.hip
+++ b/willow-inference-server_amd/csrc/dec_kernels.hip
@@ -1920,7 +1920,7 @@
 __device__ __forceinline__ bool better_b(float av, int ai, float bv, int bi) { return (av > bv) | ((av == bv) & (ai < bi)); }
 __device__ __forceinline__ void take_better(float& v, int& i, float ov, int oi) { const bool t = better_b(ov, oi, v, i); v = t ? ov : v; i = t ? oi : i; }
 
-template <bool TS>
+template <bool TS, bool BEGIN = true>
 __global__ __launch_bounds__(256) void logit_stats_kernel(const float* __restrict__ logits, const float* __restrict__ bias_all,
                                                           const float* __restrict__ bias_begin, const int* __restrict__ step_u,
                                                           float* __restrict__ st_max, float* __restrict__ st_sum,
@@ -1937,7 +1937,7 @@
   const int lo = sc * SL, hi = (lo + SL < cfg.n_vocab) ? lo + SL : cfg.n_vocab;
   const int jb = m - b * cfg.beam;
   const float* row = logits + (size_t)(b * lr_b + (rowmap ? rowmap[jb] : jb) * lr_j + lr_off) * cfg.n_vocab_pad;
-  const bool first = (step == 0) && cfg.suppress_blank;
+  const bool first = BEGIN && (step == 0) && cfg.suppress_blank;
   const bool mask_eot = cfg.fixed_new > 0 && step < cfg.fixed_new;
   const bool force_eot = cfg.fixed_new > 0 && step >= cfg.fixed_new;
 
@@ -1952,14 +1952,16 @@
   for (int i = 0; i < PT; ++i) {
     const int nidx = lo + lane + 64 * i;
     const int cidx = nidx < hi ? nidx : hi - 1;
-    lv[i] = row[cidx]; lb[i] = bias_begin[cidx]; la[i] = bias_all ? bias_all[cidx] : 0.f;
+    lv[i] = row[cidx];
+    if constexpr (BEGIN) lb[i] = bias_begin[cidx]; else lb[i] = 0.f;
+    la[i] = bias_all ? bias_all[cidx] : 0.f;
   }
   float mx = -INFINITY;
 #pragma unroll
   for (int i = 0; i < PT; ++i) {
     const int nidx = lo + lane + 64 * i;
     float v = lv[i] + la[i];
-    v = first ? v + lb[i] : v;
+    if constexpr (BEGIN) v = first ? v + lb[i] : v;
     bool dead = (nidx >= hi) | (mask_eot & (nidx == cfg.eot)) | (force_eot & (nidx != cfg.eot));
     if constexpr (TS) dead = dead | ((nidx >= r0l) & (nidx < r0h)) | ((nidx >= r1l) & (nidx < r1h)) | ((nidx >= r2l) & (nidx < r2h));
     v = dead ? -INFINITY : v;
@@ -1995,8 +1997,13 @@
 }
 int launch_logit_stats(hipStream_t st, const float* logits, const float* bias_all, const float* bias_begin, const int* step_u,
                        float* st_max, float* st_sum, float* st_val, int* st_idx, int B, const SampleCfg& cfg, int lr_b, int lr_j, int lr_off,
-                       unsigned long long* prof, const int* rowmap, const int* ts_desc) {
+                       unsigned long long* prof, const int* rowmap, const int* ts_desc, bool past_first) {
   if (cdiv(cfg.n_vocab, STAT_SUB) > 16 * 64) { set_error("logit_stats: vocab too large"); return WIS_E_UNSUPPORTED; }
+  if (past_first && !ts_desc) {
+    hipLaunchKernelGGL((logit_stats_kernel<false, false>), dim3(STAT_SUB / 4, B * cfg.beam), dim3(256), 0, st, logits, bias_all, bias_begin, step_u,
+                       st_max, st_sum, st_val, st_idx, cfg, lr_b, lr_j, lr_off, prof, rowmap, nullptr);
+    return WIS_OK;
+  }
   if (ts_desc) hipLaunchKernelGGL(logit_stats_kernel<true>, dim3(STAT_SUB / 4, B * cfg.beam), dim3(256), 0, st, logits, bias_all, bias_begin, step_u,
                                   st_max, st_sum, st_val, st_idx, cfg, lr_b, lr_j, lr_off, prof, rowmap, ts_desc);
   else hipLaunchKernelGGL(logit_stats_kernel<false>, dim3(STAT_SUB / 4, B * cfg.beam), dim3(256), 0, st, logits, bias_all, bias_begin, step_u,
@@ -2183,10 +2190,42 @@
   __hip_atomic_store(bs.host + HP_REC, rec, __ATOMIC_RELEASE, __HIP_MEMORY_SCOPE_SYSTEM);
 }
 
+constexpr int STEP_ROWS_EU = 8;
+__device__ __forceinline__ void step_rows_item(int e, int k, int d4, float inv_d4, int* j, int* c4) {
+  int jj = (int)(((float)e + 0.5f) * inv_d4);
+  jj = jj < k ? jj : k - 1;
+  *j = jj; *c4 = e - jj * d4;
+}
+__device__ __forceinline__ void step_rows_issue(const StepRows& sr, const int* nb_tok, int npos, int k, int base, int tid, f16x4 (&ea)[STEP_ROWS_EU], f16x4 (&eb)[STEP_ROWS_EU]) {
+  const int d4 = sr.d >> 2, n4 = k * d4;
+  const float inv_d4 = 1.0f / (float)d4;
+#pragma unroll
+  for (int u = 0; u < STEP_ROWS_EU; ++u) {
+    const int e = base + tid + 256 * u;
+    int j, c4; step_rows_item(e < n4 ? e : n4 - 1, k, d4, inv_d4, &j, &c4);
+    ea[u] = *reinterpret_cast<const f16x4*>(sr.emb + (size_t)nb_tok[j] * sr.d + 4 * c4);
+    eb[u] = *reinterpret_cast<const f16x4*>(sr.pos_emb + (size_t)npos * sr.d + 4 * c4);
+  }
+}
+__device__ __forceinline__ void step_rows_store(const StepRows& sr, int r0, int k, int base, int tid, const f16x4 (&ea)[STEP_ROWS_EU], const f16x4 (&eb)[STEP_ROWS_EU]) {
+  const int d4 = sr.d >> 2, n4 = k * d4;
+  const float inv_d4 = 1.0f / (float)d4;
+#pragma unroll
+  for (int u = 0; u < STEP_ROWS_EU; ++u) {
+    const int e = base + tid + 256 * u;
+    if (e < n4) {
+      int j, c4; step_rows_item(e, k, d4, inv_d4, &j, &c4);
+      const float4 v = make_float4((float)ea[u][0] + (float)eb[u][0], (float)ea[u][1] + (float)eb[u][1], (float)ea[u][2] + (float)eb[u][2], (float)ea[u][3] + (float)eb[u][3]);
+      *reinterpret_cast<float4*>(sr.x + (size_t)(r0 + j) * sr.d + 4 * c4) = v;
+      if (sr.xh) { const f16x4 h = {(f16)v.x, (f16)v.y, (f16)v.z, (f16)v.w}; *reinterpret_cast<f16x4*>(sr.xh + (size_t)(r0 + j) * sr.d + 4 * c4) = h; }
+    }
+  }
+}
+
 template <int PSL>
 __global__ __launch_bounds__(256) void beam_step_kernel(const float* __restrict__ st_max, const float* __restrict__ st_sum,
                                                         const float* __restrict__ st_val, const int* __restrict__ st_idx,
-                                                        BeamState bs, RowMeta rm, int P, int ctx, SampleCfg cfg, unsigned long long* prof) {
+                                                        BeamState bs, RowMeta rm, int P, int ctx, SampleCfg cfg, unsigned long long* prof, StepRows sr) {
   constexpr int HPT = (MAX_R * 256 + 255) / 256;
   __shared__ float lse[MAX_R], s_cum[MAX_R];
   __shared__ float cand_v[MAX_CAND]; __shared__ int cand_word[MAX_CAND]; __shared__ int cand_org[MAX_CAND];
@@ -2348,6 +2387,8 @@
     return;
   }
   stamp(pf, 7);
+  f16x4 ea[STEP_ROWS_EU], eb[STEP_ROWS_EU];
+  if (sr.emb) step_rows_issue(sr, nb_tok, npos, k, 0, tid, ea, eb);
   for (int j = 0; j < k; ++j) {
     const int org = cand_org[nb_src[j]];
     int* al = bs.alive + (size_t)(r0 + j) * cfg.max_new;
@@ -2363,15 +2404,27 @@
     }
   }
   if (tid == 0) bs.step_u[b] = step + 1;
+  if (sr.emb) {
+    const int n4 = k * (sr.d >> 2);
+    for (int base = 0;;) {
+      step_rows_store(sr, r0, k, base, tid, ea, eb);
+      base += 256 * STEP_ROWS_EU;
+      if (base >= n4) break;
+      step_rows_issue(sr, nb_tok, npos, k, base, tid, ea, eb);
+    }
+  }
   __syncthreads();
+  stamp(pf, 8);
   if (tid == 0) publish_step(bs);
-  stamp(pf, 8);
+  stamp(pf, 9);
 }
 int launch_beam_step(hipStream_t st, const float* st_max, const float* st_sum, const float* st_val, const int* st_idx,
-                     const BeamState& bs, const RowMeta& rm, int B, int P, int ctx, const SampleCfg& cfg, unsigned long long* prof) {
+                     const BeamState& bs, const RowMeta& rm, int B, int P, int ctx, const SampleCfg& cfg, unsigned long long* prof, const StepRows& sr) {
   if (cfg.beam > MAX_R || cfg.n_cand > MAX_CAND || cfg.max_new > 256 || ctx > 512 || cfg.n_vocab > (1 << 20)) { set_error("beam_step: config out of range"); return WIS_E_UNSUPPORTED; }
-  if (cfg.beam * STAT_SUB * cfg.n_cand <= 16 * 256) hipLaunchKernelGGL(beam_step_kernel<16>, dim3(B), dim3(256), 0, st, st_max, st_sum, st_val, st_idx, bs, rm, P, ctx, cfg, prof);
-  else hipLaunchKernelGGL(beam_step_kernel<32>, dim3(B), dim3(256), 0, st, st_max, st_sum, st_val, st_idx, bs, rm, P, ctx, cfg, prof);
+  if (sr.emb && (!sr.pos_emb || !sr.x || sr.d < 4 || sr.d % 4 || sr.d > 2048 || P < 1 || P - 1 + cfg.max_new > ctx || B * cfg.beam > MAX_ROWS)) {
+    set_error("beam_step: next-pass rows of d = %d at P = %d, max_new = %d, ctx = %d unsupported", sr.d, P, cfg.max_new, ctx); return WIS_E_UNSUPPORTED; }
+  if (cfg.beam * STAT_SUB * cfg.n_cand <= 16 * 256) hipLaunchKernelGGL(beam_step_kernel<16>, dim3(B), dim3(256), 0, st, st_max, st_sum, st_val, st_idx, bs, rm, P, ctx, cfg, prof, sr);
+  else hipLaunchKernelGGL(beam_step_kernel<32>, dim3(B), dim3(256), 0, st, st_max, st_sum, st_val, st_idx, bs, rm, P, ctx, cfg, prof, sr);
   return WIS_OK;
 }
 
diff --git a/willow-inference-server_amd/csrc/generate.hip b/willow-inference-server_amd/csrc/generate.hip
--- a/willow-inference-server_amd/csrc/generate.hip
+++ b/willow-inference-server_amd/csrc/generate.hip
@@ -97,7 +97,7 @@
 }
 
 struct LogitRows { int b, j, off; };
-enum { TAIL_TAPS = 1, TAIL_NO_CACHE = 2 };
+enum { TAIL_TAPS = 1, TAIL_NO_CACHE = 2, TAIL_STEP_ROWS = 4, TAIL_PAST_FIRST = 8 };
 static int sampling_tail(const SampleCtx& g, LogitRows rows, int flags) {
   wis_model* m = g.m; hipStream_t st = g.st; const wis_config_t& c = m->cfg;
   const int lr_b = rows.b, lr_j = rows.j, lr_off = rows.off;
@@ -105,8 +105,9 @@
   if (g.rep()) WIS_RET(launch_rep_rules(st, m->logits, m->bs, g.B, g.sc, g.rep_pen, g.rep_ngram, lr_b, lr_j, lr_off));
   if (g.ts) WIS_RET(launch_ts_rules(st, m->logits, g.bias_all, m->bias_begin, m->bs, g.B, g.sc, c.no_timestamps, g.ts_max_init, lr_b, lr_j, lr_off, m->ts_desc));
   WIS_RET(launch_logit_stats(st, m->logits, g.bias_all, m->bias_begin, m->bs.step_u, m->st_max, m->st_sum, m->st_val, m->st_idx, g.B, g.sc, lr_b, lr_j, lr_off, prof ? prof + 16 : nullptr,
-                             nullptr, g.ts ? m->ts_desc : nullptr));
-  WIS_RET(launch_beam_step(st, m->st_max, m->st_sum, m->st_val, m->st_idx, m->bs, m->rm, g.B, g.P, c.n_text_ctx, g.sc, prof));
+                             nullptr, g.ts ? m->ts_desc : nullptr, (flags & TAIL_PAST_FIRST) != 0));
+  WIS_RET(launch_beam_step(st, m->st_max, m->st_sum, m->st_val, m->st_idx, m->bs, m->rm, g.B, g.P, c.n_text_ctx, g.sc, prof,
+                           (flags & TAIL_STEP_ROWS) ? step_rows(m, g.B * g.beam) : StepRows()));
   if (!(flags & TAIL_NO_CACHE)) WIS_RET(launch_kv_reorder(st, m->kc_all, m->vc_all, m->kv_layer_stride, c.n_dec_layers, m->bs, g.B, g.beam, g.P, c.n_text_ctx, c.d_model));
   return WIS_OK;
 }
@@ -140,7 +141,7 @@
   wis_model* m = g.m; const wis_config_t& c = m->cfg; const int B = g.B, P = g.P;
   WIS_RET(dec_forward(m, B * P, P, B, true, g.beam, 0));
   if (g.sot_row >= 0) WIS_RET(launch_no_speech(g.st, m->logits, m->n_vocab_pad, B, P, g.sot_row, c.n_vocab, c.no_speech, m->d_nsp));
-  return sampling_tail(g, {P, 0, P - 1}, TAIL_TAPS);
+  return sampling_tail(g, {P, 0, P - 1}, TAIL_TAPS | TAIL_STEP_ROWS);
 }
 
 static int fill_tree_window(const int* hd, int s0, int Rw, int k, int P, std::vector<int>& tok, std::vector<int>& pos, std::vector<int>& slot, std::vector<int>& ls, int* ha) {
@@ -227,6 +228,7 @@
     if (sd->steps < 1) { set_error("wis_generate_draft_beam: verification completed no step"); return WIS_E_STATE; }
     WIS_RET(reseed_tick(m, sd->steps));
     WIS_HIP_CHECK(hipMemsetAsync(m->bs.done, 0, 4, st));
+    WIS_RET(embed_step_rows(m, beam));
   }
   return WIS_OK;
 }
@@ -291,6 +293,7 @@
     WIS_HIP_CHECK(hipMemcpyAsync(m->rm.lslot, &hw.slot, 4, hipMemcpyHostToDevice, st));
     WIS_HIP_CHECK(hipMemcpyAsync(m->bs.cum, &hw.cum, 4, hipMemcpyHostToDevice, st));
     WIS_RET(reseed_tick(m, steps));
+    WIS_RET(embed_step_rows(m, 1));
   }
   return WIS_OK;
 }
@@ -305,8 +308,8 @@
     return !sa_short ? 8 : (len <= 16 ? 2 : (len <= 32 ? 4 : 8));
   }
   int one_step() const {
-    WIS_RET(dec_forward(g.m, g.B * g.beam, g.beam, g.B, true, g.beam, 1));
-    return sampling_tail(g, {g.beam, 1, 0}, TAIL_TAPS);
+    WIS_RET(dec_forward(g.m, g.B * g.beam, g.beam, g.B, true, g.beam, 1, nullptr, step_rows(g.m, g.B * g.beam).emb != nullptr));
+    return sampling_tail(g, {g.beam, 1, 0}, TAIL_TAPS | TAIL_STEP_ROWS | TAIL_PAST_FIRST);
   }
   int graph_for(int nb, hipGraphExec_t* out) const {
     wis_model* m = g.m; const SampleCfg& sc = g.sc;
diff --git a/willow-inference-server_amd/csrc/kernels.hpp b/willow-inference-server_amd/csrc/kernels.hpp
--- a/willow-inference-server_amd/csrc/kernels.hpp
+++ b/willow-inference-server_amd/csrc/kernels.hpp
@@ -117,7 +117,8 @@
                        float* st_max, float* st_sum, float* st_val, int* st_idx, int B, const SampleCfg& cfg,
                        int lr_b, int lr_j, int lr_off, unsigned long long* prof = nullptr,
                        const int* rowmap = nullptr,
-                       const int* ts_desc = nullptr);
+                       const int* ts_desc = nullptr,
+                       bool past_first = false);
 constexpr int TS_DESC_INTS = 8;
 struct BeamState;
 int launch_ts_rules(hipStream_t st, const float* logits, const float* bias_all, const float* bias_begin, const BeamState& bs, int B,
@@ -153,8 +154,10 @@
 __host__ __device__ inline float* hp_out_score(unsigned long long* hp) { return reinterpret_cast<float*>(hp + HP_WORDS) + HP_MAXB; }
 __host__ __device__ inline int* hp_out_ids(unsigned long long* hp) { return reinterpret_cast<int*>(hp + HP_WORDS) + 2 * HP_MAXB; }
 int launch_kv_reorder(hipStream_t st, f16* kc, f16* vc, size_t layer_stride, int L, const BeamState& bs, int B, int beam, int P, int ctx, int d);
+struct StepRows { const f16* emb = nullptr; const f16* pos_emb = nullptr; float* x = nullptr; f16* xh = nullptr; int d = 0; };
 int launch_beam_step(hipStream_t st, const float* st_max, const float* st_sum, const float* st_val, const int* st_idx,
-                     const BeamState& bs, const RowMeta& rm, int B, int P, int ctx, const SampleCfg& cfg, unsigned long long* prof = nullptr);
+                     const BeamState& bs, const RowMeta& rm, int B, int P, int ctx, const SampleCfg& cfg, unsigned long long* prof = nullptr,
+                     const StepRows& sr = StepRows());
 constexpr int DRAFT_VS_INTS = 32 + MAX_R * 32, DRAFT_VS_PERM = 8, DRAFT_VS_BASE = 16;
 int launch_draft_match(hipStream_t st, const BeamState& bs, const int* draft, int n_draft, int beam, int* vstate, int book);
 int launch_kv_gather(hipStream_t st, f16* kc, f16* vc, size_t layer_stride, int L, const int* vstate, const int* done, int beam, int w0, int ctx, int d);
diff --git a/willow-inference-server_amd/csrc/model.hip b/willow-inference-server_amd/csrc/model.hip
--- a/willow-inference-server_amd/csrc/model.hip
+++ b/willow-inference-server_amd/csrc/model.hip
@@ -812,7 +812,7 @@
   return {frag, m->cq_fold, ln_ok && ln_f16 && d <= 2048};
 }
 
-int dec_forward(wis_model* m, int M, int R, int B, bool want_logits, int sstride, int rmul, const TreeWin* tw = nullptr) {
+int dec_forward(wis_model* m, int M, int R, int B, bool want_logits, int sstride, int rmul, const TreeWin* tw = nullptr, bool rows_ready = false) {
   const wis_config_t& c = m->cfg; hipStream_t st = m->st;
   const int d = c.d_model, H = c.n_heads, T = c.n_audio_ctx, ctx = c.n_text_ctx;
   static const int env_chunks = getenv("WIS_CROSS_CHUNKS") ? atoi(getenv("WIS_CROSS_CHUNKS")) : 0;
@@ -823,7 +823,7 @@
   const bool fold = rt.fold, ln16 = rt.ln16;
   const int ln = ln16 ? GV_LN16 : GV_LN;
   auto ln_x = [&](const f16* x16) { return ln16 ? (const void*)x16 : (const void*)m->dx; };
-  WIS_RET(launch_dec_embed(st, m->emb, m->dec_pos, m->rm.tok, m->rm.pos, m->dx, M, d, fold ? m->dxh : nullptr));
+  if (!rows_ready) WIS_RET(launch_dec_embed(st, m->emb, m->dec_pos, m->rm.tok, m->rm.pos, m->dx, M, d, fold ? m->dxh : nullptr));
   SelfAttnP sa;
   sa.q = m->dq; sa.pos = m->rm.pos; sa.out = m->dao; sa.M = M; sa.H = H; sa.d = d; sa.ctx = ctx; sa.rpu = R; sa.sstride = sstride; sa.rmul = rmul; sa.nb = m->sa_nb;
   CrossAttnP ca;
@@ -870,6 +870,19 @@
   }
   if (want_logits) WIS_RET(launch_gemv(st, gemv_small(m->proj, ln_x(m->dxh), m->logits, M, ln | GV_OUT_F32)));
   return WIS_OK;
+}
+
+static StepRows step_rows(const wis_model* m, int M) {
+  StepRows sr;
+  const StepRoute rt = small_route(m, M);
+  if (rt.frag || m->cfg.d_model % 4 || m->cfg.d_model > 2048) return sr;
+  sr.emb = m->emb; sr.pos_emb = m->dec_pos; sr.x = m->dx; sr.xh = rt.fold ? m->dxh : nullptr; sr.d = m->cfg.d_model;
+  return sr;
+}
+static int embed_step_rows(wis_model* m, int M) {
+  const StepRoute rt = small_route(m, M);
+  if (!step_rows(m, M).emb) return WIS_OK;
+  return launch_dec_embed(m->st, m->emb, m->dec_pos, m->rm.tok, m->rm.pos, m->dx, M, m->cfg.d_model, rt.fold ? m->dxh : nullptr);
 }
 
 static int init_beam_state(wis_model* m, int B, int beam) {
diff --git a/willow-inference-server_amd/csrc/taps.hip b/willow-inference-server_amd/csrc/taps.hip
--- a/willow-inference-server_amd/csrc/taps.hip
+++ b/willow-inference-server_amd/csrc/taps.hip
@@ -582,4 +582,52 @@
   return t.finish(launch_greedy_pick(t.st, smax, ssum, sval, sidx, rows, sc, tok_out, lp_out));
 }
 
-}
+int wis_debug_tail_rows(wis_model_t* m, const float* logits, int n_steps, int B, int P, const wis_gen_opts_t* o, int stats_form, const float* bias_begin,
+                        uint32_t fill_x, uint16_t fill_xh, int32_t* out_tok, int32_t* out_pos, int32_t* out_done, float* out_x, uint16_t* out_xh,
+                        float* out_st_max, float* out_st_sum, float* out_st_val, int32_t* out_st_idx) {
+  if (!m || !logits || !o || n_steps < 1 || n_steps > MAX_STEPS || P < 1 || P > 16 || stats_form < 0 || stats_form > 1) { set_error("wis_debug_tail_rows: bad argument"); return WIS_E_ARG; }
+  WIS_ENTER(m, "wis_debug_tail_rows")
+  WIS_HIP_CHECK(hipSetDevice(m->device));
+  Tap t(m->device, "wis_debug_tail_rows"); WIS_RET(t.rc);
+  const wis_config_t& c = m->cfg; hipStream_t st = m->st;
+  const int beam = o->beam_size < 1 ? 1 : o->beam_size;
+  WIS_RET(check_batch(m, B, beam));
+  WIS_RET(check_patience(beam, o->patience));
+  const int max_new = o->max_new_tokens > 0 ? std::min(o->max_new_tokens, MAX_STEPS) : n_steps;
+  if (max_new < n_steps || P - 1 + max_new > c.n_text_ctx) { set_error("wis_debug_tail_rows: %d steps at prompt length %d, max_new_tokens %d, %d text positions", n_steps, P, max_new, c.n_text_ctx); return WIS_E_ARG; }
+  if (o->timestamps || o->repetition_penalty != 0.f || o->no_repeat_ngram_size != 0) { set_error("wis_debug_tail_rows: the plain tail only"); return WIS_E_UNSUPPORTED; }
+  const int Mrows = B * beam, V = c.n_vocab, d = c.d_model;
+  float* bb = nullptr;
+  if (bias_begin) {
+    WIS_RET(t.get(&bb, (size_t)m->n_vocab_pad, true));
+    WIS_HIP_CHECK(hipStreamSynchronize(t.st));
+    WIS_HIP_CHECK(hipMemcpyAsync(bb, bias_begin, (size_t)V * 4, hipMemcpyHostToDevice, st));
+  }
+  float patience;
+  SampleCfg sc = make_sample_cfg(m, o, beam, max_new, &patience);
+  const float* bias_all = o->suppress_default ? m->bias_all : nullptr;
+  WIS_RET(init_beam_state(m, B, beam));
+  StepRows sr; sr.emb = m->emb; sr.pos_emb = m->dec_pos; sr.x = m->dx; sr.xh = m->dxh; sr.d = d;
+  const size_t nst = (size_t)Mrows * STAT_SUB;
+  for (int s = 0; s < n_steps; ++s) {
+    WIS_HIP_CHECK(hipMemcpy2DAsync(m->logits, (size_t)m->n_vocab_pad * 4, logits + (size_t)s * Mrows * V, (size_t)V * 4, (size_t)V * 4, Mrows, hipMemcpyHostToDevice, st));
+    WIS_HIP_CHECK(hipMemsetD32Async(reinterpret_cast<hipDeviceptr_t>(m->dx), (int)fill_x, (size_t)Mrows * d, st));
+    WIS_HIP_CHECK(hipMemsetD16Async(reinterpret_cast<hipDeviceptr_t>(m->dxh), (unsigned short)fill_xh, (size_t)Mrows * d, st));
+    WIS_RET(launch_logit_stats(st, m->logits, bias_all, bb ? bb : m->bias_begin, m->bs.step_u, m->st_max, m->st_sum, m->st_val, m->st_idx, B, sc, beam, s == 0 ? 0 : 1, 0,
+                               nullptr, nullptr, nullptr, stats_form == 0 && s > 0));
+    WIS_RET(launch_beam_step(st, m->st_max, m->st_sum, m->st_val, m->st_idx, m->bs, m->rm, B, P, c.n_text_ctx, sc, nullptr, sr));
+    if (out_tok) WIS_HIP_CHECK(hipMemcpyAsync(out_tok + (size_t)s * Mrows, m->rm.tok, (size_t)Mrows * 4, hipMemcpyDeviceToHost, st));
+    if (out_pos) WIS_HIP_CHECK(hipMemcpyAsync(out_pos + (size_t)s * Mrows, m->rm.pos, (size_t)Mrows * 4, hipMemcpyDeviceToHost, st));
+    if (out_done) WIS_HIP_CHECK(hipMemcpyAsync(out_done + (size_t)s * B, m->bs.done, (size_t)B * 4, hipMemcpyDeviceToHost, st));
+    if (out_x) WIS_HIP_CHECK(hipMemcpyAsync(out_x + (size_t)s * Mrows * d, m->dx, (size_t)Mrows * d * 4, hipMemcpyDeviceToHost, st));
+    if (out_xh) WIS_HIP_CHECK(hipMemcpyAsync(out_xh + (size_t)s * Mrows * d, m->dxh, (size_t)Mrows * d * 2, hipMemcpyDeviceToHost, st));
+    if (out_st_max) WIS_HIP_CHECK(hipMemcpyAsync(out_st_max + s * nst, m->st_max, nst * 4, hipMemcpyDeviceToHost, st));
+    if (out_st_sum) WIS_HIP_CHECK(hipMemcpyAsync(out_st_sum + s * nst, m->st_sum, nst * 4, hipMemcpyDeviceToHost, st));
+    if (out_st_val) WIS_HIP_CHECK(hipMemcpyAsync(out_st_val + s * nst * sc.n_cand, m->st_val, nst * sc.n_cand * 4, hipMemcpyDeviceToHost, st));
+    if (out_st_idx) WIS_HIP_CHECK(hipMemcpyAsync(out_st_idx + s * nst * sc.n_cand, m->st_idx, nst * sc.n_cand * 4, hipMemcpyDeviceToHost, st));
+    WIS_HIP_CHECK(hipStreamSynchronize(st));
+  }
+  return t.finish(WIS_OK);
+}
+
+}
diff --git a/willow-inference-server_amd/wis_hip/_lib.py b/willow-inference-server_amd/wis_hip/_lib.py
--- a/willow-inference-server_amd/wis_hip/_lib.py
+++ b/willow-inference-server_amd/wis_hip/_lib.py
@@ -132,6 +132,7 @@
     ("wis_op_no_speech", _i, [_i, _vp, _i, _i, _i, _i, _i, _i, _vp]),
     ("wis_op_lang_probs", _i, [_i, _vp, _i, _vp, _i, _vp, _i]),
     ("wis_op_greedy_rows", _i, [_i, _vp, _i, _i, _i, _vp, _vp, _vp, _i, _i, _i, _i, _i, _vp, _vp, _vp]),
+    ("wis_debug_tail_rows", _i, [_vp, _vp, _i, _i, _i, C.POINTER(GenOpts), _i, _vp, C.c_uint32, C.c_uint16] + [_vp] * 9),
     ("wis_sv_create", _i, [C.POINTER(SvConfig), _vp, _sz, _i, C.POINTER(Tensor), _i, _i, C.POINTER(_vp)]),
     ("wis_sv_destroy", None, [_vp]),
     ("wis_sv_device_bytes", _sz, [_vp]),
```

Result: no change. 151.0 x realtime (-0.2%).
